# lh3/ksw2

Measured on AMD Instinct MI355X. Metric: GCUPS (DP cells/s) + pairs/s at fixed (qlen,tlen,band), higher is better.
Workload: dtype int16x2 (packed, two alignments per lane); 1 GPU; 10k: 49152 pairs/step/GPU, qlen=10000 tlen=10000 band=500 zdrop=400 extz2 affine score-only; setup_priming_batches=0, parallelism=pairs sharded over 1 GPU(s), one process per GPU, no collective in the data path

## Files before the change

### ksw2_amd/csrc/ksw2_host_plan.c

```c
#include "ksw2_host_int.h"


__thread char g_err[512];
__thread int g_no_defer;
static __thread int g_probe_tasks;
size_t thread_cached_device_bytes(void);

const char *ksw2amd_last_error(void) { return g_err; }
const char *ksw2amd_backend(void) { return k2a_shim_backend(); }
int ksw2amd_device_count(void) { return k2a_shim_device_count(); }


void ksw2amd_release_cache(void);

static const char *const g_env_name[ENV_COUNT] = {
#define X(n) "KSW2AMD_" #n,
	K2A_ENV_LIST
#undef X
};
__thread void *g_plan_stream;
__thread int g_latency_plan;
const char *g_env[ENV_COUNT];
volatile int g_env_ready;
static int g_env_gen;
// ... 234 lines not shown
	ez->n_cigar = 0; ez->zdropped = 0; ez->reach_end = 0;
}

void ez_reserve(void *km, ksw_extz_t *ez, int n)
{
	int m = ez->m_cigar;
	if (n <= m) return;
	while (m < n) m = m ? m << 1 : 4;
	ez->cigar = (uint32_t*)cigar_realloc(km, ez->cigar, (size_t)m << 2);
	ez->m_cigar = m;
}






int64_t band_cells(int qlen, int tlen, int w)
{
	const int64_t T = (int64_t)qlen + w < tlen ? (int64_t)qlen + w : tlen;
	const int64_t a = (int64_t)qlen - 1 - w;
	const int64_t na = a < 0 ? 0 : (a + 1 < T ? a + 1 : T);
	const int64_t nb = (int64_t)w + 1 < T ? (int64_t)w + 1 : T;
	const int64_t sum_en = na * (na - 1) / 2 + na * w + (T - na) * ((int64_t)qlen - 1);
	const int64_t sum_st = (T - nb) * (T - 1 + nb) / 2 - (T - nb) * (int64_t)w;
	return T <= 0 ? 0 : sum_en - sum_st + T;
}

static size_t mp_total_steps(int G, int C, int qlen, int tlen, int w)
{
	const int R = G * C, ngen = (tlen + R - 1) / R;
	size_t tot = 0;
	int g;
	for (g = 0; g < ngen; ++g) {
		const int lo = imax(0, g * R - w), hi = imin(qlen - 1, imin(g * R + R - 1, tlen - 1) + w);
		const int nl = imin(G, (tlen - g * R + C - 1) / C);
		if (hi >= lo) tot += ((size_t)(hi - lo + 1) + (size_t)(nl - 1) + 7) & ~(size_t)7;
		(void)0;
	}
	return tot;
}

int geom_fits(int G, int C, int tlen_eff, int w)
{
	const int nstrips = (tlen_eff + C - 1) / C;
	return nstrips <= G || 2 * (int64_t)w < (int64_t)G * (C + 1) - C + 1;
}

static int cfg_fits(int cfg, int tlen_eff, int w)
{
	if (cfg == K2A_CFG_MP) return 1;
	return geom_fits(k2a_cfg_G[cfg], k2a_cfg_C[cfg], tlen_eff, w);
}

void build_eff(int dual, int m, const int8_t *mat, int e, int e2, int generic, int8_t *eff)
{
	int a, b;
	if (generic) memcpy(eff, mat, (size_t)m * m);
	else {
		int scN = mat[m * m - 1] == 0 ? -(dual ? e2 : e) : mat[m * m - 1];
		for (a = 0; a < m; ++a)
			for (b = 0; b < m; ++b)
				eff[a * m + b] = (int8_t)((a == m - 1 || b == m - 1) ? scN : a == b ? mat[0] : mat[1]);
	}
}

static void build_scoring(int dual, int m, const int8_t *mat, int q, int e, int q2, int e2, int generic, K2aScoring *sc)
{
	int8_t eff[K2A_MAXM * K2A_MAXM];
	int a, b;
	memset(sc, 0, sizeof(*sc));
	sc->q = q; sc->e = e; sc->q2 = dual ? q2 : 0; sc->e2 = dual ? e2 : 0;
	sc->m = m;
	build_eff(dual, m, mat, e, e2, generic, eff);
	if (m > 5) return;
	for (a = 0; a < m; ++a) {
		uint32_t p = 0;
		for (b = 0; b < 4 && b < m; ++b) p |= (uint32_t)(uint8_t)eff[a * m + b] << (8 * b);
		sc->prof[a] = p;
		sc->colw[a] = m == 5 ? eff[a * m + 4] : 0;
	}
}

typedef struct { int ok, smax, smin, qemax, qemin, q, e, tn1; uint32_t cp[8]; } pkinfo_t;

static void pk_scoring(int dual, int m, const int8_t *mat, int q, int e, int q2, int e2, int generic, pkinfo_t *o)
{
	int8_t eff[25];
	int x, y, ok = (m >= 1 && m <= 5);
	memset(o, 0, sizeof(*o));
	if (ok) {
		build_eff(dual, m, mat, e, e2, generic, eff);
		o->smax = o->smin = eff[0];
		for (x = 0; x < m * m; ++x) { o->smax = imax(o->smax, eff[x]); o->smin = imin(o->smin, eff[x]); }
		for (y = 0; y < m; ++y)
			for (x = 0; x < 4 && x < m; ++x) o->cp[y] |= (uint32_t)(o->smax - eff[x * m + y]) << (8 * x);
		if (m == 5 && !(ENV(TN) && ENV(TN)[0] == '0')) {
			for (y = 1; y < 5 && eff[4 * 5 + y] == eff[4 * 5]; ++y) {}
			if (y == 5) o->tn1 = o->smax - eff[4 * 5] + 1;
		}
	}
	o->q = q; o->e = e;
	o->qemax = dual ? imax(q + e, q2 + e2) : q + e;
	o->qemin = dual ? imin(q + e, q2 + e2) : q + e;
	if (q < 0 || e < 0 || (dual && (q2 < 0 || e2 < 0)) || o->smax + e < 0) ok = 0;
	o->ok = ok;
}

static int pk_eligible(const pkinfo_t *k, int qlen, int tlen, int w)
{
	const int64_t L = imin(qlen, tlen);
	int64_t hmax, hmin;
	if (k->ok <= 0 || qlen > 32000 || tlen > 32000) return 0;
	hmax = (int64_t)imax(k->smax, 0) * L + (int64_t)k->e * tlen;
	hmin = -((int64_t)k->q + (int64_t)k->e * (w + 1)) + (int64_t)imin(k->smin, 0) * L;
	return hmax < K2A_PK_VMAX - 2 * k->qemax - 8 && hmin > K2A_NEG16 + 2 * k->qemax + 8;
}

static int pk_window_ok(const pkinfo_t *k, int qlen, int tlen, int w, int C)
{
	const int64_t D = imax(imax(k->smax, 0) + k->qemin, -k->smin) + k->e;
	if (k->ok <= 0 || qlen > 65000 || tlen > 65000) return 0;
	if ((int64_t)4 * C * D + 2 * k->qemax + imax(k->smax, 0) + (k->smax - k->smin) + 64 > K2A_PK_SLACK) return 0;
	return ((int64_t)2 * w + 2 * C + 2) * D + 2 * k->qemax + (int64_t)4 * C * D + 64 <= 12000;
}

static int pk_slide_ok(const pkinfo_t *k, int qlen, int tlen)
{
	const int64_t D = imax(imax(k->smax, 0) + k->qemin, -k->smin) + k->e;
	if (k->ok <= 0 || qlen > 65000 || tlen > 65000) return 0;
	if (K2A_PKMP_RMAX_LIMIT + (K2A_PKMP_T + 4) * D + 2 * k->qemax + 64 > K2A_PK_VMAX) return 0;
	return (K2A_PKMP_T + 2 * 16 + 4) * D + 2 * k->qemax + 64 <= 6000;
}

static inline uint64_t above4(uint64_t v) { return ((v >> 3 | v >> 4 | v >> 5 | v >> 6 | v >> 7) | ((v >> 2) & (v | (v >> 1)))) & 0x0101010101010101ull; }

int copy_scan(uint8_t *dst, const uint8_t *src, int n)
{
	int i = 0;
	uint64_t acc = 0, hi = 0, v0, v1, v2, v3;
	for (; i + 32 <= n; i += 32) {
		memcpy(&v0, src + i, 8); memcpy(&v1, src + i + 8, 8); memcpy(&v2, src + i + 16, 8); memcpy(&v3, src + i + 24, 8);
		memcpy(dst + i, &v0, 8); memcpy(dst + i + 8, &v1, 8); memcpy(dst + i + 16, &v2, 8); memcpy(dst + i + 24, &v3, 8);
		acc |= (v0 | v1) | (v2 | v3);
		if (((v0 | v1) | (v2 | v3)) & 0x0404040404040404ull) hi |= (above4(v0) | above4(v1)) | (above4(v2) | above4(v3));
	}
	for (; i < n; ++i) { dst[i] = src[i]; acc |= src[i]; if (src[i] > 4) hi = 1; }
	return (acc & 0xf8f8f8f8f8f8f8f8ull) || hi ? 2 : (acc & 0x0404040404040404ull) ? 1 : 0;
}

void ksw2amd_plan_destroy(ksw2amd_plan_t *p)
{
	int i;
	if (!p) return;
	if (p->gather) gather_wait(p);
	if (p->up_ev) { k2a_shim_event_sync(p->up_ev); k2a_shim_event_destroy(p->up_ev); p->up_ev = 0; }
	if (p->up_state) {
		int k;
		for (k = 0; k < K2A_MAXPIECES; ++k) if (p->up_state->ev2[k]) k2a_shim_event_destroy(p->up_state->ev2[k]);
		pthread_mutex_destroy(&p->up_state->mu); free(p->up_state); p->up_state = 0;
	}
	if (p->wm_ev) { k2a_shim_event_destroy(p->wm_ev); p->wm_ev = 0; }
	if (p->meta_ev) { k2a_shim_event_sync(p->meta_ev); k2a_shim_event_destroy(p->meta_ev); p->meta_ev = 0; }
	if (p->stream_used) k2a_shim_stream_sync(p->stream);
	cache_put(BUF_SEQ, p->d_seq, p->cap[BUF_SEQ]); cache_put(BUF_TB, p->d_tb, p->cap[BUF_TB]);
	if (p->meta_folded != 2) cache_put(BUF_PAIRS, p->d_pairs, p->cap[BUF_PAIRS]);
	cache_put(BUF_RES, p->d_res, p->cap[BUF_RES]);
	if (!p->meta_folded) cache_put(BUF_ORDER, p->d_order, p->cap[BUF_ORDER]);
	cache_put(BUF_CIG, p->d_cig, p->cap[BUF_CIG]);
	cache_put(BUF_BND, p->d_bnd, p->cap[BUF_BND]); cache_put(BUF_WM, p->d_wm, p->cap[BUF_WM]); cache_put(BUF_HMETA, p->h_meta, p->cap[BUF_HMETA]);
	cache_put(BUF_PK4, p->d_pk4, p->cap[BUF_PK4]);
	free(p->h_qd);
	for (i = 0; i < 3; ++i) if (p->ev[i]) { if (!g_ev_cache[i]) g_ev_cache[i] = p->ev[i]; else k2a_shim_event_destroy(p->ev[i]); }
	free(p->h_pairs); free(p->h_cls); free(p->h_half); free(p->h_flag); free(p->h_order);
	cache_put(BUF_HRES, p->h_res, p->cap[BUF_HRES]);
	if (!p->flat) cache_put(BUF_HSEQ, p->h_seq, p->cap[BUF_HSEQ]);
	free(p->src_pairs); free(p->src_mat); free(p->flat_tail); free(p->uni);
	free(p);
}

int cmp_cost_desc(const void *a, const void *b)
{
// ... 343 lines not shown
		const char *ev = ENV(SIMDS);
		const int simds = ev ? atoi(ev) : k2a_shim_simd_count();
		if (simds > 0) {
			int cnt[NCLS_MAX * NPASS], b;
			memset(cnt, 0, sizeof(cnt));
			if (uni) { if (p->h_cls[0] >= 0 && pk_ok[0] && pk_ok[0] != PASS_SOLO) cnt[p->h_cls[0] * NPASS + pk_ok[0]] = g_probe_tasks ? 2 * g_probe_tasks : n; }
			else
			for (i = 0; i < n; ++i) if (p->h_cls[i] >= 0 && pk_ok[i] && pk_ok[i] != PASS_SOLO) ++cnt[p->h_cls[i] * NPASS + pk_ok[i]];
			for (b = 0; b < NCLS_MAX * NPASS; ++b)
				if (cnt[b]) {
					const int pcb = (b % NPASS - 1) % K2A_NPKCFG, G = k2a_pkcfg_G[pcb];
					const int64_t waves = ((int64_t)(cnt[b] + 1) / 2 * G + 63) / 64 * (pcb == K2A_PKCFG_MP ? 4 : 1);
					cnt[b] = G != 64 ? 0 : (solo_mode == 3 && pcb != K2A_PKCFG_MP && cnt[b] <= simds ? 2 : 0) | (waves * 10 < (int64_t)simds * 4 ? 1 : 0);
				}
			if (uni && !(p->h_cls[0] >= 0 && pk_ok[0] && pk_ok[0] != PASS_SOLO && cnt[p->h_cls[0] * NPASS + pk_ok[0]])) {  }
			else
			for (i = 0; i < n; ++i)
				if (p->h_cls[i] >= 0 && pk_ok[i] && pk_ok[i] != PASS_SOLO) {
					const int what = cnt[p->h_cls[i] * NPASS + pk_ok[i]];
					if ((what & 2) && solo_ok[i]) pk_ok[i] = PASS_SOLO;
					else if (what & 1) pk_ok[i] = 0;
				}
		}
	}

	if (tlev) tph[3] = now_ms();
	if (m > 5 && !flat && !su) {
		build_eff(dual, m, sc->mat, e, e2, 0, (int8_t*)p->h_seq + mat_off);
		build_eff(dual, m, sc->mat, e, e2, 1, (int8_t*)p->h_seq + mat_off + (size_t)m * m);
	}
	if (!su && !g_probe_tasks) p->d_seq = (uint8_t*)cache_get(BUF_SEQ, p->seq_bytes + (flat ? 0 : META_ROOM(n)), &p->cap[BUF_SEQ]);
	if (!p->d_seq && !g_probe_tasks) { fail(KSW2AMD_E_NOMEM, "device allocation failed: %s", k2a_shim_last_error()); goto err; }
	up = su ? su->up : (flat && !flat->on_device) || (!flat && p->seq_bytes >= ((size_t)(ENV(SHARED_UP_MIN_MB) ? imax(atoi(ENV(SHARED_UP_MIN_MB)), 0) : 4) << 20) && !ENV(NO_SHARED_UP)) ? shared_upload_stream() : 0;
	if (up) shared_up = 1; else up = g_plan_stream ? g_plan_stream : thread_upload_stream();
	p->stream = up; p->stream_used = !g_probe_tasks;
	if (su) {  }
	else if (flat) {
		const size_t tail = p->seq_bytes - flat_span;
		flat_tmp = (uint8_t*)calloc(tail ? tail : 1, 1);
		if (!flat_tmp) { fail(KSW2AMD_E_NOMEM, "plan_create: host allocation failed%s", 0); goto err; }
		if (m > 5) {
			build_eff(dual, m, sc->mat, e, e2, 0, (int8_t*)flat_tmp + (mat_off - flat_span));
			build_eff(dual, m, sc->mat, e, e2, 1, (int8_t*)flat_tmp + (mat_off - flat_span) + (size_t)m * m);
		}
	}

	{
		enum { NB = NCLS_MAX * NPASS };
		int bcnt[NB], bpos[NB], b;
		p->ncls = 0; p->ntasks = 0;
		p->h_order = (uint32_t*)malloc(sizeof(uint32_t) * (3 * (size_t)n + 4));
		srt = (sort_t*)malloc(sizeof(sort_t) * ((size_t)n + 1));
		if (!p->h_order || !srt) { fail(KSW2AMD_E_NOMEM, "plan_create: host allocation failed%s", 0); goto err; }
		memset(bcnt, 0, sizeof(bcnt));
		if (uni) bcnt[p->h_cls[0] * NPASS + pk_ok[0]] = n;
		else
		for (i = 0; i < n; ++i) if (p->h_cls[i] >= 0) ++bcnt[p->h_cls[i] * NPASS + pk_ok[i]];
		for (b = 0, k = 0; b < NB; ++b) { bpos[b] = k; k += bcnt[b]; }
		if (uni) { for (b = 0; b < NB; ++b) bpos[b] += bcnt[b]; }
		else
		for (i = 0; i < n; ++i)
			if (p->h_cls[i] >= 0) {
				sort_t *e_ = &srt[bpos[p->h_cls[i] * NPASS + pk_ok[i]]++];
				e_->idx = (uint32_t)i;
				e_->cost = ((int64_t)p->h_pairs[i].qlen << 40) + ((int64_t)p->h_pairs[i].tlen << 16) + p->h_pairs[i].w;
				e_->tf = (uint32_t)p->h_pairs[i].tlen_full;
			}
		for (b = 0, k = 0; b < NB; ++b) {
			const int cnt = bcnt[b], pass = b % NPASS;
			sort_t *g = srt + (bpos[b] - cnt);
			int ntask = 0;
			cls_t *c;
			if (cnt == 0) continue;
			ci = b / NPASS;
			if (!uni) {
			for (i = 1; i < cnt && cmp_cost_desc(&g[i - 1], &g[i]) <= 0; ++i) {}
			if (i < cnt) qsort(g, (size_t)cnt, sizeof(sort_t), cmp_cost_desc);
			}
			c = &p->cls[p->ncls++];
			c->solo = pass == PASS_SOLO;
			c->cfg = c->solo ? 0 : pass ? (pass - 1) % K2A_NPKCFG : ci / 6; c->rb = pass && !c->solo ? ((pass - 1) / K2A_NPKCFG) & 1 : 0;
			c->nomax = !c->solo && pass > 2 * K2A_NPKCFG; c->mode = (ci / 2) % 3; c->generic = ci & 1; c->pk = pass != 0 && !c->solo; c->first = k;
			build_scoring(dual, m, sc->mat, q, e, q2, e2, c->generic, &c->sc);
			if (pkinfo[c->generic].ok > 0) { memcpy(c->sc.cp, pkinfo[c->generic].cp, sizeof(c->sc.cp)); c->sc.pk_smax = pkinfo[c->generic].smax; c->sc.pk_tn1 = pkinfo[c->generic].tn1; }
			if (uni) {
				if (!pass || c->solo) { for (i = 0; i < cnt; ++i) p->h_order[k++] = (uint32_t)i; ntask = cnt; }
				else for (i = 0; i < cnt; i += 2, ++ntask) { p->h_order[k++] = (uint32_t)i; p->h_order[k++] = (uint32_t)(i + 1 < cnt ? i + 1 : i); }
			} else
			if (!pass || c->solo) {
				for (i = 0; i < cnt; ++i) p->h_order[k++] = g[i].idx;
				ntask = cnt;
			} else {
				for (i = 0; i < cnt; ++ntask) {
					const uint32_t ia = g[i].idx;
					uint32_t ib = ia;
					if (i + 1 < cnt && g[i + 1].cost == g[i].cost && g[i + 1].tf == g[i].tf) { ib = g[i + 1].idx; i += 2; } else i += 1;
					p->h_order[k++] = ia; p->h_order[k++] = ib;
				}
			}
			c->count = ntask;
			p->ntasks += ntask;
		}
		p->norder = k;
		free(srt); srt = 0;
	}

	if (tlev) tph[4] = now_ms();
	for (k = 0; k < p->ncls; ++k) {
		const cls_t *c = &p->cls[k];
		if (!c->pk || c->cfg != K2A_PKCFG_MP) continue;
		for (i = 0; i < c->count; ++i) {
			K2aPair *da = &p->h_pairs[p->h_order[c->first + 2 * i]], *db = &p->h_pairs[p->h_order[c->first + 2 * i + 1]];
			p->bnd_words = align_up(p->bnd_words, 4);
			da->bnd_off = db->bnd_off = (uint32_t)p->bnd_words;
			p->bnd_words += align_up((size_t)da->qlen * (dual ? 5 : 4) + 16, 4) + K2A_PKMP_WAVES * (size_t)(64 * 16 * 2 * 2);
			if (p->bnd_words > 0xfff00000u) { fail(KSW2AMD_E_PARAM, "plan_create: boundary rows over 16 GiB in one plan%s", 0); goto err; }
		}
	}

	{
		const char *ev = ENV(DEFER);
		const int forced = ev && *ev ? (atoi(ev) != 0) : -1;
		size_t ck_total = 0;
		for (k = 0; k < p->ncls; ++k) {
			cls_t *c = &p->cls[k];
			c->defer = c->pk && !c->solo && c->cfg != K2A_PKCFG_MP && !dual && c->mode == K2A_MODE_SCORE && !c->nomax && !g_no_defer &&
			           (forced < 0 ? k2a_pkcfg_G[c->cfg] == 64 && (k2a_shim_simd_count() > 0 ? 2 * (int64_t)(g_probe_tasks ? g_probe_tasks : c->count) >= 3 * (int64_t)k2a_shim_simd_count()
			                                                                                      : (g_probe_tasks ? g_probe_tasks : c->count) >= 32) : forced);
		}
		if (g_probe_tasks) { free(pk_ok); free(solo_ok); return p; }
		for (lo = 0; lo < 2; ++lo) {
			size_t at = p->tb_bytes;
			for (k = 0; k < p->ncls; ++k) {
				const cls_t *c = &p->cls[k];
				const int G = c->pk ? k2a_pkcfg_G[c->cfg] : 64, C = c->pk ? k2a_pkcfg_C[c->cfg] : 16, NG = 64 / G;
				int t0;
				if (!c->defer) continue;
				at += align_up(4 * K2A_ZLIST_WORDS(c->count), 256);
				for (t0 = 0; t0 < c->count; t0 += NG) {
					uint32_t steps = 0, hs = 0;
					int t;
					size_t bytes;
					for (t = t0; t < imin(c->count, t0 + NG); ++t) {
						const K2aPair *d = &p->h_pairs[p->h_order[c->first + 2 * t]];
						const uint32_t ns = (uint32_t)((d->tlen + C - 1) / C);
						steps = (uint32_t)imax((int)steps, (int)ns - 1 + imin(d->qlen - 1, d->tlen - 1 + d->w) + 1);
						hs = (uint32_t)imax((int)hs, (int)ns);
					}
					bytes = align_up((size_t)steps * 512 + (size_t)NG * hs * 16, 256);
					if (lo) for (t = t0; t < imin(c->count, t0 + NG); ++t) {
						K2aPair *da = &p->h_pairs[p->h_order[c->first + 2 * t]], *db = &p->h_pairs[p->h_order[c->first + 2 * t + 1]];
						da->tb_off = db->tb_off = at; da->bnd_off = db->bnd_off = steps; da->cig_off = db->cig_off = hs;
					}
					at += bytes;
				}
			}
			if (!lo) {
				ck_total = at - p->tb_bytes;
				if (ck_total > ((size_t)1 << 30) && forced < 0) {
					size_t free_b = 0, total_b = 0;
					if (k2a_shim_mem_info(&free_b, &total_b) || ck_total > (free_b + thread_cached_device_bytes()) / 10 * 6) {
						for (k = 0; k < p->ncls; ++k) p->cls[k].defer = 0;
						ck_total = 0;
						break;
					}
				}
				if (ck_total == 0) break;
// ... 439 lines not shown
	}
	if (k2a_shim_event_record(p->ev[1], stream)) goto err;
	for (c = 0; c < p->ncls; ++c) {
		const cls_t *k = &p->cls[c];
		if (k->mode == K2A_MODE_SCORE || (streaming && k->qd >= 0)) continue;
		if (k->solo) {
			if (k2a_shim_launch_trace_solo(p->d_pairs, p->d_order + k->first, k->count, p->d_tb, p->d_res, p->d_cig, stream)) goto err;
		} else if (k->pk) {
			if (k2a_shim_launch_trace_pk(k->cfg, p->dual, p->d_pairs, p->d_order + k->first, k->count, p->d_tb, p->d_res, p->d_cig, stream)) goto err;
		} else if (k2a_shim_launch_trace(k->cfg, p->dual, p->d_pairs, p->d_order + k->first, k->count, p->d_tb, p->d_res, p->d_cig, stream)) goto err;
	}
	if (k2a_shim_event_record(p->ev[2], stream)) goto err;
	return KSW2AMD_OK;
err:
	return fail(KSW2AMD_E_NODEVICE, "plan_run: %s", k2a_shim_last_error());
}

int ksw2amd_plan_timing(ksw2amd_plan_t *p, float *fill_ms, float *total_ms)
{
	if (!p || !p->ran) return fail(KSW2AMD_E_PARAM, "plan_timing: plan has not run%s", 0);
	if (p->reject_all || p->ntasks == 0) { if (fill_ms) *fill_ms = 0; if (total_ms) *total_ms = 0; return KSW2AMD_OK; }
	if (fill_ms) *fill_ms = k2a_shim_event_ms(p->ev[0], p->ev[1]);
	if (total_ms) *total_ms = k2a_shim_event_ms(p->ev[0], p->ev[2]);
	return KSW2AMD_OK;
}

int64_t ksw2amd_plan_cells(const ksw2amd_plan_t *p) { return p ? p->cells : 0; }
int64_t ksw2amd_plan_packed_pairs(const ksw2amd_plan_t *p)
{
	int64_t n = 0;
	int c, i;
	if (!p) return 0;
	for (c = 0; c < p->ncls; ++c)
		if (p->cls[c].pk)
			for (i = 0; i < p->cls[c].count; ++i)
				n += p->h_order[p->cls[c].first + 2 * i] == p->h_order[p->cls[c].first + 2 * i + 1] ? 1 : 2;
		else if (p->cls[c].solo) n += p->cls[c].count;
	return n;
}
int ksw2amd_plan_describe(const ksw2amd_plan_t *p, char *buf, int cap)
{
	static const char *const mode_name[3] = { "score", "left", "right" }, *const form_name[4] = { "registers", "ldsrows", "ldscodes", "defer" };
	int c, len = 0;
	if (!p || !buf || cap <= 0) return 0;
	buf[0] = 0;
	if (p->splice == 2 && !p->reject_all) {
		static const char *const fkind[10] = { "extf-lds", "extf-lds", "extf-lds", "extf-hbm", "extf-win4", "extf-win8", "extf-lane", "extf-grp", "extf-grp32", "extf-grp64" };
		int nl = 0;
		for (c = 0; c < 10 && len < cap - 1; ++c)
			if (p->f_count[c]) {
				len += snprintf(buf + len, (size_t)(cap - len), "kernel=%s form=%s ring=%d tasks=%d\n", fkind[c], c == 6 && p->f_par.ring ? "ldsring" : c == 6 ? "hbm" : "-",
				                c == 6 ? p->f_par.ring : 0, p->f_count[c]);
				++nl;
			}
		return nl;
	}
	if (p->splice == 1 && !p->reject_all) {
		static const char *const skind[3] = { "exts-win8", "exts-win16", "exts-hbm" };
		int nl = 0, mode, g, wn;
		for (mode = 0; mode < 3; ++mode) for (g = 0; g < 2; ++g) for (wn = 0; wn < 3 && len < cap - 1; ++wn)
			if (p->s_count[mode][g][wn]) {
				len += snprintf(buf + len, (size_t)(cap - len), "kernel=%s mode=%s generic=%d tasks=%d\n", skind[wn], mode_name[mode], g, p->s_count[mode][g][wn]);
				++nl;
			}
		return nl;
	}
	if (p->splice == 3 && !p->reject_all) {
		static const char *const form_name[3] = { "hbm", "lds", "blk" };
		int nl = 0, mode, lds;
		for (mode = 0; mode < 3; ++mode) for (lds = 0; lds < 3 && len < cap - 1; ++lds)
			if (p->s_count[mode][0][lds]) {
				len += snprintf(buf + len, (size_t)(cap - len), "kernel=ssec gaps=%d mode=%s form=%s tasks=%d\n", p->dual ? 2 : 1, mode_name[mode], form_name[lds], p->s_count[mode][0][lds]);
				++nl;
			}
		return nl;
	}
	if (p->splice || p->reject_all) return 0;
	for (c = 0; c < p->ncls && len < cap - 1; ++c) {
		const cls_t *k = &p->cls[c];
		const char *kind = k->solo ? "solo" : k->pk ? (k->cfg == K2A_PKCFG_MP ? "pkmp" : "pk") : (k->cfg == K2A_CFG_MP ? "mp" : "int32");
		const int G = k->solo ? 64 : k->pk ? k2a_pkcfg_G[k->cfg] : k2a_cfg_G[k->cfg], C = k->solo ? 2 * K2A_SOLO_ROWS(k->mode == K2A_MODE_SCORE) : k->pk ? k2a_pkcfg_C[k->cfg] : k2a_cfg_C[k->cfg];
		const int form = k->defer ? 3 : k->solo ? 0 : k->pk ? (k->cfg == K2A_PKCFG_MP ? 0 : k2a_shim_pk_form(k->cfg, p->dual, k->mode, k->nomax, k->count))
		                                     : (k->cfg == K2A_CFG_MP ? k2a_shim_mp_form(p->dual, k->mode, k->count) : 0);
		len += snprintf(buf + len, (size_t)(cap - len), "kernel=%s G=%d C=%d gaps=%d mode=%s rebased=%d nomax=%d generic=%d form=%s tasks=%d uniform=%d wire4=%d tn=%d\n",
		                kind, G, C, p->dual ? 2 : 1, mode_name[k->mode], k->rb, k->nomax, k->generic, form_name[form], k->count, p->uni ? 1 : 0,
		                p->up_state ? p->up_state->wire4 : 0, (k->pk || k->solo) && k->sc.pk_tn1 ? 1 : 0);
	}
	return p->ncls;
}
int64_t ksw2amd_plan_device_bytes(const ksw2amd_plan_t *p)
{
	if (!p) return 0;
	return (int64_t)(p->seq_bytes + p->tb_bytes + p->cig_words * 4 + p->bnd_words * 4 + (sizeof(K2aPair) + sizeof(K2aResult)) * (size_t)p->n + 4 * (size_t)p->norder);
}

static int fetch_results(ksw2amd_plan_t *p)
{
	if (!p || !p->ran) return fail(KSW2AMD_E_PARAM, "plan_fetch: plan has not run%s", 0);
	if (p->gather && gather_wait(p)) return fail(KSW2AMD_E_NODEVICE, "plan_fetch: upload failed: %s", k2a_shim_last_error());
	if (p->reject_all || p->ntasks == 0) return KSW2AMD_OK;
	if (p->streamed && p->nqd > 0) {
		if (k2a_shim_stream_sync(p->stream)) return fail(KSW2AMD_E_NODEVICE, "plan_fetch: %s", k2a_shim_last_error());
		K2aQueueDesc back[NCLS_ENTRIES];
		int k, aborted = 0;
		if (k2a_shim_d2h(back, p->d_wm + K2A_WM_BYTES, sizeof(K2aQueueDesc) * (size_t)p->nqd, p->stream) || k2a_shim_stream_sync(p->stream))
			return fail(KSW2AMD_E_NODEVICE, "plan_fetch: %s", k2a_shim_last_error());
		for (k = 0; k < p->nqd; ++k) aborted |= back[k].abort != 0 || back[k].next < back[k].nwt;
		if (aborted) {
			void *st = p->stream;
			__sync_fetch_and_add(&g_stream_stat[1], 1);
			if (trace_level()) fprintf(stderr, "[ksw2_amd] streamed plan n=%d: a launch gave up waiting for its inputs (abort %u, started %u of %u wavefront-tasks, %d pieces); running the plan again behind its upload\n", p->n, back[0].abort, back[0].next, back[0].nwt, p->npieces);
			p->streamed = 0;
			if ((p->up_ev && k2a_shim_event_sync(p->up_ev)) || k2a_shim_memset(p->d_res, 0, sizeof(K2aResult) * (size_t)p->n, st) ||
			    (plan_wire4(p) && k2a_shim_launch_wire_expand(p->d_pk4, p->d_seq, (size_t)p->uni->n * p->uni->stride, plan_wire4(p), p->uni->stride, st)) ||
			    ksw2amd_plan_run(p, st) || k2a_shim_stream_sync(st))
				return fail(KSW2AMD_E_NODEVICE, "plan_fetch: %s", k2a_shim_last_error());
		}
	}
	if (k2a_shim_d2h(p->h_res, p->d_res, sizeof(K2aResult) * (size_t)p->n, p->stream) ||
	    k2a_shim_stream_sync(p->stream))
		return fail(KSW2AMD_E_NODEVICE, "plan_fetch: %s", k2a_shim_last_error());
	return KSW2AMD_OK;
}

int64_t g_reruns;
int64_t ksw2amd_rerun_count(void) { return g_reruns; }
int ksw2amd_plan_fetch_raw(ksw2amd_plan_t *p, int32_t *out16)
{
	int i, rc = fetch_results(p);
	if (rc) return rc;
	memset(out16, 0, sizeof(int32_t) * 16 * (size_t)p->n);
	for (i = 0; i < p->n; ++i)
		if (!p->reject_all && needs_rerun(p, i)) {
			ksw_extz_t z;
			int32_t *o = out16 + 16 * (size_t)i;
			memset(&z, 0, sizeof(z));
			rc = pair_rerun(p, i, 0, &z);
			if (rc) { free(z.cigar); return rc; }
			o[0] = (int32_t)z.max; o[1] = (int32_t)z.zdropped; o[2] = z.max_q; o[3] = z.max_t; o[4] = z.mqe; o[5] = z.mqe_t; o[6] = z.mte; o[7] = z.mte_q;
			o[8] = z.score; o[9] = z.reach_end; o[10] = z.n_cigar; o[11] = p->h_res[i].rows_done; o[12] = o[13] = -1;
			free(z.cigar);
		} else if (p->h_cls[i] >= 0 && !p->reject_all) memcpy(out16 + 16 * (size_t)i, &p->h_res[i], sizeof(K2aResult));
		else {
			int32_t *o = out16 + 16 * (size_t)i;
			o[2] = o[3] = o[5] = o[7] = -1; o[4] = o[6] = o[8] = KSW_NEG_INF; o[12] = o[13] = -1;
		}
	return KSW2AMD_OK;
}

void eqx_rewrite(void *km, const uint8_t *query, const uint8_t *target, int stride, ksw_extz_t *ez)
{
	int n0 = ez->n_cigar, k, i, x = 0, y = 0, n = 0;
	uint32_t *old = (uint32_t*)malloc(sizeof(uint32_t) * (size_t)(n0 + 1));
	memcpy(old, ez->cigar, sizeof(uint32_t) * (size_t)n0);
	ez->n_cigar = 0;
	for (k = 0; k < n0; ++k) {
		uint32_t op = old[k] & 0xf, len = old[k] >> 4;
		if (op == KSW_CIGAR_MATCH) {
			for (i = 0; i < (int)len; ++i) {
				uint32_t o = target[(size_t)(x + i) * stride] == query[(size_t)(y + i) * stride] ? KSW_CIGAR_EQ : KSW_CIGAR_X;
				if (n > 0 && (ez->cigar[n - 1] & 0xf) == o) ez->cigar[n - 1] += 1u << 4;
				else { ez_reserve(km, ez, n + 1); ez->cigar[n++] = 1u << 4 | o; }
			}
			x += (int)len; y += (int)len;
		} else {
			if (n > 0 && (ez->cigar[n - 1] & 0xf) == op) ez->cigar[n - 1] += len << 4;
			else { ez_reserve(km, ez, n + 1); ez->cigar[n++] = len << 4 | op; }
			if (op == KSW_CIGAR_DEL || op == KSW_CIGAR_N_SKIP) x += (int)len;
			else if (op == KSW_CIGAR_INS) y += (int)len;
// ... 292 lines not shown
```

### ksw2_amd/csrc/ksw2_lane_pk.h

```cpp
#ifndef KSW2_LANE_PK_H_
#define KSW2_LANE_PK_H_

#include "ksw2_lane.h"
#include "ksw2_lane_rowmask.h"

#define K2A_PK_STAGE(C) (3 * (C) + 4)
typedef uint32_t k2a_pk;
#define K2A_OFS   (K2A_OFS16 * 0x10001u)

K2A_FN k2a_pk k2a_pk2(int v) { return ((uint32_t)v & 0xffffu) | ((uint32_t)v << 16); }
K2A_FN int k2a_pk_lo(k2a_pk v) { return (int)(int16_t)(v & 0xffffu); }
K2A_FN int k2a_pk_hi(k2a_pk v) { return (int)(int16_t)(v >> 16); }
K2A_FN k2a_pk k2a_pk_sel(k2a_pk m, k2a_pk a, k2a_pk b) { return (m & a) | (~m & b); }
K2A_FN k2a_pk k2a_pair16(uint32_t lo, uint32_t hi) { return lo | (hi << 16); }
K2A_FN k2a_pk k2a_byte_pair(uint32_t a, uint32_t b, int r)
{
#if defined(__HIP_DEVICE_COMPILE__)
	return __builtin_amdgcn_perm(b, a, 0x0c040c00u + (uint32_t)r * 0x00010001u);
#else
	return ((a >> (8 * r)) & 0xffu) | (((b >> (8 * r)) & 0xffu) << 16);
#endif
}
K2A_FN uint32_t k2a_perm(uint32_t s0, uint32_t s1, uint32_t sel)
{
// ... 16 lines not shown
}
#define K2A_TSEL_BASE 0x0c040c00u
K2A_FN uint32_t k2a_h16(int v) { return (uint32_t)(v + K2A_OFS16) & 0xffffu; }
K2A_FN k2a_pk k2a_pku(int v) { return k2a_pk2(v + K2A_OFS16); }
K2A_FN k2a_pk k2a_add32(k2a_pk a, k2a_pk b) { return a + b; }
K2A_FN k2a_pk k2a_sub32(k2a_pk a, k2a_pk b) { return a - b; }

#if defined(__HIP_DEVICE_COMPILE__)
typedef short k2a_s2 __attribute__((ext_vector_type(2)));
typedef unsigned short k2a_u2 __attribute__((ext_vector_type(2)));
K2A_FN k2a_pk k2a_pk_add(k2a_pk a, k2a_pk b) { return __builtin_bit_cast(k2a_pk, (k2a_s2)(__builtin_bit_cast(k2a_s2, a) + __builtin_bit_cast(k2a_s2, b))); }
K2A_FN k2a_pk k2a_pk_sub(k2a_pk a, k2a_pk b) { return __builtin_bit_cast(k2a_pk, (k2a_s2)(__builtin_bit_cast(k2a_s2, a) - __builtin_bit_cast(k2a_s2, b))); }
K2A_FN k2a_pk k2a_pk_max(k2a_pk a, k2a_pk b) { return __builtin_bit_cast(k2a_pk, __builtin_elementwise_max(__builtin_bit_cast(k2a_s2, a), __builtin_bit_cast(k2a_s2, b))); }
K2A_FN k2a_pk k2a_pk_min(k2a_pk a, k2a_pk b) { return __builtin_bit_cast(k2a_pk, __builtin_elementwise_min(__builtin_bit_cast(k2a_s2, a), __builtin_bit_cast(k2a_s2, b))); }
K2A_FN k2a_pk k2a_pk_maxu(k2a_pk a, k2a_pk b) { return __builtin_bit_cast(k2a_pk, __builtin_elementwise_max(__builtin_bit_cast(k2a_u2, a), __builtin_bit_cast(k2a_u2, b))); }
K2A_FN k2a_pk k2a_pk_max3u(k2a_pk a, k2a_pk b, k2a_pk c)
{
	k2a_pk d;
	asm("v_pk_maximum3_f16 %0, %1, %2, %3" : "=v"(d) : "v"(a), "v"(b), "v"(c));
	return d;
}
K2A_FN k2a_pk k2a_pk_mad(k2a_pk a, k2a_pk b, k2a_pk c)
{
	k2a_pk d;
	asm("v_pk_mad_i16 %0, %1, %2, %3" : "=v"(d) : "v"(a), "v"(b), "v"(c));
	return d;
}
K2A_FN k2a_pk k2a_pk_sign(k2a_pk a)
{
	k2a_pk d;
	asm("v_pk_ashrrev_i16 %0, 15, %1 op_sel_hi:[0,1]" : "=v"(d) : "v"(a));
	return d;
}
K2A_FN k2a_pk k2a_pk_selv(k2a_pk m, k2a_pk a, k2a_pk b)
{
	k2a_pk d;
	asm("v_bitop3_b32 %0, %1, %2, %3 bitop3:0xe4" : "=v"(d) : "v"(a), "v"(b), "v"(m));
	return d;
}
K2A_FN k2a_pk k2a_pk_shl(k2a_pk a, int n)
{
	return n == 0 ? a : __builtin_bit_cast(k2a_pk, (k2a_u2)(__builtin_bit_cast(k2a_u2, a) << (k2a_u2)(unsigned short)n));
}
K2A_FN k2a_pk k2a_bit_mask(uint32_t bits, int c) { return (k2a_pk)__builtin_amdgcn_sbfe((int)bits, c, 1); }
#define K2A_SCHED_FENCE() __builtin_amdgcn_sched_barrier(0)
K2A_FN uint32_t k2a_load_early(const uint8_t *p) { uint32_t v; __builtin_memcpy(&v, p, 4); return v; }
#else
#define K2A_SCHED_FENCE() do {} while (0)
K2A_FN uint32_t k2a_load_early(const uint8_t *p) { uint32_t v; __builtin_memcpy(&v, p, 4); return v; }
K2A_FN k2a_pk k2a_pk_mk(int lo, int hi) { return ((uint32_t)lo & 0xffffu) | ((uint32_t)hi << 16); }
K2A_FN k2a_pk k2a_pk_add(k2a_pk a, k2a_pk b) { return k2a_pk_mk(k2a_pk_lo(a) + k2a_pk_lo(b), k2a_pk_hi(a) + k2a_pk_hi(b)); }
K2A_FN k2a_pk k2a_pk_sub(k2a_pk a, k2a_pk b) { return k2a_pk_mk(k2a_pk_lo(a) - k2a_pk_lo(b), k2a_pk_hi(a) - k2a_pk_hi(b)); }
K2A_FN k2a_pk k2a_pk_max(k2a_pk a, k2a_pk b) { return k2a_pk_mk(k2a_max(k2a_pk_lo(a), k2a_pk_lo(b)), k2a_max(k2a_pk_hi(a), k2a_pk_hi(b))); }
K2A_FN k2a_pk k2a_pk_min(k2a_pk a, k2a_pk b) { return k2a_pk_mk(k2a_min(k2a_pk_lo(a), k2a_pk_lo(b)), k2a_min(k2a_pk_hi(a), k2a_pk_hi(b))); }
K2A_FN k2a_pk k2a_pk_maxu(k2a_pk a, k2a_pk b)
{
	const uint32_t al = a & 0xffffu, ah = a >> 16, bl = b & 0xffffu, bh = b >> 16;
	return (al > bl ? al : bl) | ((ah > bh ? ah : bh) << 16);
}
K2A_FN k2a_pk k2a_pk_max3u(k2a_pk a, k2a_pk b, k2a_pk c)
{
	uint32_t r = 0;
	for (int h = 0; h < 2; ++h) {
		const uint32_t x = (a >> (16 * h)) & 0xffffu, y = (b >> (16 * h)) & 0xffffu, z = (c >> (16 * h)) & 0xffffu;
		uint32_t m = x > y ? x : y;
		m = m > z ? m : z;
		if (m > 0x7BFFu) m = 0x7BFFu - (m & 0xffu);
		r |= m << (16 * h);
	}
	return r;
}
K2A_FN k2a_pk k2a_pk_mad(k2a_pk a, k2a_pk b, k2a_pk c) { return k2a_pk_mk(k2a_pk_lo(a) * k2a_pk_lo(b) + k2a_pk_lo(c), k2a_pk_hi(a) * k2a_pk_hi(b) + k2a_pk_hi(c)); }
K2A_FN k2a_pk k2a_pk_sign(k2a_pk a) { return ((a & 0x8000u) ? 0xffffu : 0u) | ((a & 0x80000000u) ? 0xffff0000u : 0u); }
K2A_FN k2a_pk k2a_pk_selv(k2a_pk m, k2a_pk a, k2a_pk b) { return k2a_pk_sel(m, a, b); }
K2A_FN k2a_pk k2a_pk_shl(k2a_pk a, int n) { return (((a & 0xffffu) << n) & 0xffffu) | ((((a >> 16) << n) & 0xffffu) << 16); }
K2A_FN k2a_pk k2a_bit_mask(uint32_t bits, int c) { return ((bits >> c) & 1u) ? 0xffffffffu : 0u; }
#endif

K2A_FN uint32_t k2a_tsel_wild(uint32_t x)
{
	const uint32_t n = x & 0x00040004u;
	return ((x ^ n) + K2A_TSEL_BASE) | n | (n << 1);
}
K2A_FN k2a_pk k2a_tn_fix(k2a_pk cand, uint32_t sel, int tn1)
{
	const uint32_t m = (sel >> 3) & 0x00010001u;
	return cand - m * ((uint32_t)(tn1 - 1) & 0xffu);
}

#define K2A_SGN_SEL 0x09080b0au
template<bool DUAL, bool NIBBLE, bool INV>
K2A_FN uint32_t k2a_dir_flags(uint32_t s1, uint32_t s2, uint32_t s3, uint32_t s4, uint32_t x1, uint32_t x2, uint32_t x3, uint32_t x4)
{
	const uint32_t q1 = k2a_perm(s1, x1, K2A_SGN_SEL), q2 = k2a_perm(s2, x2, K2A_SGN_SEL);
	uint32_t r = k2a_pk_selv(0x55555555u, q1, q2);
	if (DUAL) {
		const uint32_t q3 = k2a_perm(s3, x3, K2A_SGN_SEL), q4 = k2a_perm(s4, x4, K2A_SGN_SEL);
		r = k2a_pk_selv(0x33333333u, r, k2a_pk_selv(0x55555555u, q3, q4));
	}
	if (INV) r = ~r;
	if (NIBBLE) return k2a_pk_selv(0x03030303u, r, r >> 16);
	const uint32_t t = k2a_pk_selv(0x0f0f0f0fu, r, r >> 16);
	return DUAL ? t : t & 0x33333333u;
}
K2A_FN uint32_t k2a_flags_decode(uint32_t b)
{
	const uint32_t win = (b & 8u) ? 4u : (b & 4u) ? 3u : (b & 2u) ? 2u : (b & 1u);
	return win | ((b >> 4) << 3);
}
K2A_FN k2a_pk k2a_ofs_on(k2a_pk plain) { return k2a_pk_add(plain, K2A_OFS); }
K2A_FN k2a_pk k2a_ofs_off(k2a_pk ofs) { return k2a_pk_sub(ofs, K2A_OFS); }

#define K2A_PK_LDSROWS(G, C, DUAL, MODE, NOMAX) ((G) == 64 && (C) == 16 && (DUAL) && (MODE) != K2A_MODE_SCORE && !(NOMAX))
#define K2A_PK_LDSROW_WORDS(C) (3 * (C) * 64)
#define K2A_PK_LDSCODES(G, C, DUAL, MODE, NOMAX) ((((G) == 64 && (C) == 16) || ((G) == 8 && (C) == 18) || ((G) == 16 && (C) == 8)) && !(DUAL) && (MODE) == K2A_MODE_SCORE)
#define K2A_PK_LDSCODE_WORDS(C) ((C) * 64)

struct K2aCkHead { int32_t baseA, baseB; uint32_t hd0, pad; };
#define K2A_CK_STEP_BYTES 512

struct K2aRowPredLane {
	uint32_t live;
	K2A_FN void begin(int dd, int w, int rows_m1)
	{
		const int lo = k2a_max(0, dd - w);
		const int hi = k2a_min(rows_m1, dd + w);
		const int cnt = k2a_max(hi - lo + 1, 0);
		live = ((1u << cnt) - 1u) << (lo & 31);
	}
	K2A_FN k2a_pk pick(int c, k2a_pk h, k2a_pk neg) const { return k2a_pk_sel(k2a_bit_mask(live, c), h, neg); }
	K2A_FN bool any() const { return live != 0; }
};
template<int C>
struct K2aRowPredUniform {
	const K2aRowMasks<C> &rm;
	int lane;
	K2A_FN K2aRowPredUniform(const K2aRowMasks<C> &rm_, int lane_) : rm(rm_), lane(lane_) {}
	K2A_FN void begin(int, int, int) {}
	K2A_FN k2a_pk pick(int c, k2a_pk h, k2a_pk neg) const
	{
#if defined(__HIP_DEVICE_COMPILE__)
		return __builtin_amdgcn_inverse_ballot_w64(rm.m[c]) ? h : neg;
#else
		return ((rm.m[c] >> lane) & 1u) ? h : neg;
#endif
	}
	K2A_FN bool any() const
	{
		uint64_t a = 0;
#pragma unroll
		for (int c = 0; c < C; ++c) a |= rm.m[c];
#if defined(__HIP_DEVICE_COMPILE__)
		return __builtin_amdgcn_inverse_ballot_w64(a);
#else
		return ((a >> lane) & 1u) != 0;
#endif
	}
};

template<int G, int C, bool DUAL, int MODE = K2A_MODE_SCORE, bool RB = false, bool NOMAX = false, int LDSROW_ = 0, bool DEFER = false, bool TN = false>
struct K2aLanePk {
	enum { NIB = K2A_PK_NIBBLES(C, DUAL), TBWORDS = NIB ? C / 4 : C / 2 };
	int qlen, tlen, tlen_full, w, nstrips;
	const uint8_t *qa, *qbp, *ta, *tbq;
	int gl, S, i0, je, koff, Snext, knext, koff_next;
	int kfin, kd, rows_m1, wup;
	k2a_pk hout, eout, e2out, hd0, hu_prev;
	int baseA, baseB;
	k2a_pk delta;
	uint32_t qb;
	uint32_t hasn;
	bool wn;
	const uint32_t *cptab;
	uint32_t cpA, cpB;
	K2A_FN void set_qb(uint32_t q) { qb = q; cpA = cptab[q & 7u]; cpB = cptab[(q >> 16) & 7u]; }
	enum { LDSROW = LDSROW_ == 1,
	       LDSTC = LDSROW_ != 0 };
	k2a_pk hl[C], f[C], f2[DUAL ? C : 1], rmax_[(NOMAX || LDSROW) ? 1 : C], rmj_[(NOMAX || LDSROW || DEFER) ? 1 : C];
	k2a_pk tc_[LDSTC ? 1 : C];
	uint32_t *lrow;
	enum { TCROW = LDSROW ? 2 : 0 };
	K2A_FN k2a_pk rmax(int c) const { return LDSROW ? lrow[(0 * C + c) * 64] : rmax_[(NOMAX || LDSROW) ? 0 : c]; }
	K2A_FN k2a_pk rmj(int c) const { return DEFER ? 0u : LDSROW ? lrow[(1 * C + c) * 64] : rmj_[(NOMAX || LDSROW) ? 0 : c]; }
	K2A_FN k2a_pk tc(int c) const { return LDSTC ? lrow[(TCROW * C + c) * 64] : tc_[LDSTC ? 0 : c]; }
	K2A_FN void set_rmax(int c, k2a_pk v) { if (LDSROW) lrow[(0 * C + c) * 64] = v; else rmax_[(NOMAX || LDSROW) ? 0 : c] = v; }
	K2A_FN void set_rmj(int c, k2a_pk v) { if (DEFER) return; if (LDSROW) lrow[(1 * C + c) * 64] = v; else rmj_[(NOMAX || LDSROW) ? 0 : c] = v; }
	K2A_FN void set_tc(int c, k2a_pk v) { if (LDSTC) lrow[(TCROW * C + c) * 64] = v; else tc_[LDSTC ? 0 : c] = v; }

	K2A_FN static int first_col(int S_, int w_) { return k2a_max(0, S_ * C - w_); }

	K2A_FN void schedule_next()
	{
		koff_next = Snext;
		knext = Snext < nstrips ? koff_next + first_col(Snext, w) : K2A_KNONE;
	}

	K2A_FN void setup(const K2aPair &pr, const K2aPair &prB, const uint8_t *seq, int lane_in_group, bool valid, const uint32_t *cptab_)
	{
		cptab = cptab_; cpA = cpB = 0;
		qlen = pr.qlen; tlen = pr.tlen; tlen_full = pr.tlen_full; w = pr.w;
		qa = seq + pr.qoff; ta = seq + pr.toff; qbp = seq + prB.qoff; tbq = seq + prB.toff;
		nstrips = valid ? (tlen + C - 1) / C : 0;
		gl = lane_in_group;
		S = -1; i0 = 0; je = -1; koff = 0; kfin = K2A_KNONE; kd = 0; rows_m1 = -1; wup = w;
		Snext = gl;
		schedule_next();
		const k2a_pk neg = k2a_pku(K2A_NEG16);
		hout = eout = e2out = hd0 = hu_prev = neg; qb = 0; qwA = qwB = 0; seen = 0;
		hasn = 0; wn = false;
		baseA = baseB = 0; delta = 0;
		local_reset();
#pragma unroll
		for (int c = 0; c < C; ++c) { hl[c] = f[c] = neg; set_tc(c, K2A_TSEL_BASE); if (!NOMAX) { set_rmax(c, neg); set_rmj(c, 0); } if (DUAL) f2[c] = neg; }
		if (NOMAX || LDSROW) rmax_[0] = neg;
		if (NOMAX || LDSROW || DEFER) rmj_[0] = 0;
		if (LDSTC) tc_[0] = 0;
		if (!DUAL) f2[0] = 0;
	}

	K2A_FN int last_step() const { return nstrips > 0 ? (nstrips - 1) + k2a_min(qlen - 1, tlen - 1 + w) : -1; }
	K2A_FN bool need_init(int k) const { return k == knext; }
	K2A_FN bool need_fin(int k) const { return k == kfin; }

	template<bool COL0U = false>
	K2A_FN void do_init(const K2aScoring &sc, int bsA = 0, int bsB = 0, const K2aCkHead *forced = 0, bool col0_any = true)
	{
		S = Snext; i0 = S * C; koff = koff_next;
		je = k2a_min(qlen - 1, k2a_min(i0 + C - 1, tlen - 1) + w);
		kfin = koff + je;
		kd = koff + i0;
		rows_m1 = k2a_min(C - 1, tlen - 1 - i0);
		wup = w + (S == 0 ? 1 : 0);
		const int js = k2a_max(0, i0 - w);
		const k2a_pk neg = k2a_pku(K2A_NEG16);
		const uint8_t *tpa = ta + (size_t)S * C, *tpb = tbq + (size_t)S * C;
		hasn = 0;
#pragma unroll
		for (int c4 = 0; c4 < C; c4 += 4) {
			uint32_t da, db;
			__builtin_memcpy(&da, tpa + c4, 4); __builtin_memcpy(&db, tpb + c4, 4);
			if (c4 + 4 > C) { da &= 0xffffu; db &= 0xffffu; }
			note_codes(da, db);
			if (TN && sc.pk_tn1 && ((da | db) & 0x04040404u)) {
				hasn = 1;
#pragma unroll
				for (int r = 0; r < 4 && c4 + r < C; ++r) set_tc(c4 + r, k2a_tsel_wild(k2a_byte_pair(da, db, r)));
			} else {
#pragma unroll
				for (int r = 0; r < 4 && c4 + r < C; ++r) set_tc(c4 + r, k2a_byte_pair(da, db, r) + K2A_TSEL_BASE);
			}
		}
#pragma unroll
		for (int c = 0; c < C; ++c) {
			hl[c] = neg; f[c] = neg; if (DUAL) f2[c] = neg;
			if (!NOMAX) set_rmax(c, neg);
		}
		const int hcorner = k2a_border<DUAL>(sc, i0) + sc.e * (i0 - 1);
		if (forced) { baseA = forced->baseA; baseB = forced->baseB; delta = 0; }
		else if (RB) {
			const int nbA = js == 0 ? hcorner : bsA + k2a_pk_lo(k2a_ofs_off(hu_prev)), nbB = js == 0 ? hcorner : bsB + k2a_pk_hi(k2a_ofs_off(hu_prev));
			delta = S == 0 ? 0u : k2a_pair16((uint32_t)(bsA - nbA) & 0xffffu, (uint32_t)(bsB - nbB) & 0xffffu);
			baseA = nbA; baseB = nbB;
		}
		if (col0_any) {
			if (COL0U) K2A_SCHED_FENCE();
			if (i0 <= w) {
#pragma unroll
				for (int c = 0; c < C; ++c) {
					const int hb = k2a_border<DUAL>(sc, i0 + c + 1) + sc.e * (i0 + c);
					if (i0 + c <= w) {
						hl[c] = k2a_ofs_on(k2a_pair16((uint32_t)(hb - baseA) & 0xffffu, (uint32_t)(hb - baseB) & 0xffffu));
						f[c] = k2a_pk_sub(hl[c], k2a_pk2(sc.q + sc.e));
						if (DUAL) f2[c] = k2a_pk_sub(hl[c], k2a_pk2(sc.q2 + sc.e2));
					}
				}
			}
		}
		if (forced) hd0 = forced->hd0;
		else if (RB) hd0 = K2A_OFS;
		else if (js == 0) hd0 = k2a_pku(hcorner);
		else hd0 = hu_prev;
		Snext += G;
		schedule_next();
	}

	K2A_FN void top_inputs(const K2aScoring &sc, int k, k2a_pk &hin, k2a_pk &ein, k2a_pk &e2in) const
	{
		if (S == 0) {
			const int hb = k2a_border<DUAL>(sc, k - koff + 1);
			const k2a_pk h0 = k2a_ofs_on(k2a_pair16((uint32_t)(hb - baseA) & 0xffffu, (uint32_t)(hb - baseB) & 0xffffu));
			hin = k2a_pk_sub(h0, k2a_pk2(sc.e));
			ein = k2a_pk_sub(h0, k2a_pk2(sc.q + sc.e)); e2in = k2a_pk_sub(h0, k2a_pk2(sc.q2 + sc.e2));
		}
	}

	K2A_FN bool step(const K2aScoring &sc, int k, k2a_pk hin, k2a_pk ein, k2a_pk e2in, uint32_t *tbw)
	{
		K2aRowPredLane rp;
		return step_rows(sc, k, hin, ein, e2in, tbw, rp);
	}

	template<class RowPred>
	K2A_FN bool step_rows(const K2aScoring &sc, int k, k2a_pk hin, k2a_pk ein, k2a_pk e2in, uint32_t *tbw, RowPred &rp)
	{
		const int dd = k - kd;
		const k2a_pk neg = k2a_pku(K2A_NEG16);
		const k2a_pk gq = k2a_pk2(sc.q), ge = k2a_pk2(sc.e), gq2 = k2a_pk2(sc.q2), ge2 = k2a_pk2(sc.e2), de2 = k2a_pk2(sc.e2 - sc.e);
		const k2a_pk bias = k2a_pk2(sc.pk_smax + sc.e);
		k2a_pk e = ein, e2 = e2in;
		if (dd >= wup) { e = neg; e2 = neg; }
		rp.begin(dd, w, rows_m1);
		const k2a_pk jjpk = k2a_pk2(k - koff);
		constexpr int CH = (C % 6 == 0) ? 6 : (C % 4 == 0) ? 4 : C;
		k2a_pk dprev = 0, uprev = 0, above_old = hd0;
#pragma unroll
		for (int c0 = 0; c0 < C; c0 += CH) {
			k2a_pk cand[CH];
			const k2a_pk last_old = hl[c0 + CH - 1];
#pragma unroll
			for (int r = 0; r < CH; ++r) {
				const int c = c0 + r;
				const k2a_pk up = r == 0 ? above_old : hl[c - 1];
				cand[r] = k2a_sub32(k2a_add32(up, bias), k2a_perm(cpB, cpA, tc(c)));
			}
			if (TN && wn) {
#pragma unroll
				for (int r = 0; r < CH; ++r) cand[r] = k2a_tn_fix(cand[r], tc(c0 + r), sc.pk_tn1);
			}
			above_old = last_old;
			if (CH < C) K2A_SCHED_FENCE();
#pragma unroll
			for (int r = 0; r < CH; ++r) {
				const int c = c0 + r;
				const k2a_pk fc = f[c];
				k2a_pk h = cand[r], s1 = 0, s2 = 0, s3 = 0, s4 = 0, x1 = 0, x2 = 0, x3 = 0, x4 = 0;
				if (MODE == K2A_MODE_SCORE) {
					h = k2a_pk_max3u(h, e, fc);
					if (DUAL) h = k2a_pk_max3u(h, e2, f2[c]);
				} else if (MODE == K2A_MODE_LEFT) {
					s1 = k2a_pk_sub(h, e);  h = k2a_pk_maxu(h, e);
					s2 = k2a_pk_sub(h, fc); h = k2a_pk_maxu(h, fc);
					if (DUAL) { s3 = k2a_pk_sub(h, e2); h = k2a_pk_maxu(h, e2); s4 = k2a_pk_sub(h, f2[c]); h = k2a_pk_maxu(h, f2[c]); }
				} else {
					s1 = k2a_pk_sub(e, h);  h = k2a_pk_maxu(h, e);
					s2 = k2a_pk_sub(fc, h); h = k2a_pk_maxu(h, fc);
					if (DUAL) { s3 = k2a_pk_sub(e2, h); h = k2a_pk_maxu(h, e2); s4 = k2a_pk_sub(f2[c], h); h = k2a_pk_maxu(h, f2[c]); }
				}
				h = rp.pick(c, h, neg);
				if (!NOMAX && DEFER) set_rmax(c, k2a_pk_maxu(rmax(c), h));
				else if (!NOMAX) {
					const k2a_pk rm = rmax(c), rj = rmj(c);
					if (!DUAL && MODE == K2A_MODE_RIGHT) set_rmj(c, k2a_pk_selv(k2a_pk_sign(k2a_pk_sub(rm, h)), jjpk, rj));
					else set_rmj(c, k2a_pk_selv(k2a_pk_sign(k2a_pk_sub(h, rm)), rj, jjpk));
					set_rmax(c, k2a_pk_maxu(rm, h));
				}
				const k2a_pk t = k2a_sub32(h, gq);
				if (MODE == K2A_MODE_LEFT) { x1 = k2a_pk_sub(t, e); x2 = k2a_pk_sub(t, fc); }
				else if (MODE == K2A_MODE_RIGHT) { x1 = k2a_pk_sub(e, t); x2 = k2a_pk_sub(fc, t); }
				e = k2a_pk_maxu(e, t);
				f[c] = k2a_sub32(k2a_pk_maxu(fc, t), ge);
				if (DUAL) {
					const k2a_pk t2 = k2a_sub32(h, gq2);
					if (MODE == K2A_MODE_LEFT) { x3 = k2a_pk_sub(t2, e2); x4 = k2a_pk_sub(t2, f2[c]); }
					else if (MODE == K2A_MODE_RIGHT) { x3 = k2a_pk_sub(e2, t2); x4 = k2a_pk_sub(f2[c], t2); }
					e2 = k2a_pk_sub(k2a_pk_maxu(e2, t2), de2);
					f2[c] = k2a_sub32(k2a_pk_maxu(f2[c], t2), ge2);
				}
				if (MODE != K2A_MODE_SCORE) {
					const uint32_t fl = k2a_dir_flags<DUAL, NIB != 0, MODE == K2A_MODE_RIGHT>(s1, s2, s3, s4, x1, x2, x3, x4);
					if (!(c & 1)) dprev = fl;
					else if (NIB) {
						const uint32_t u = k2a_pk_selv(0x0f0f0f0fu, dprev, fl << 4);
						if ((c & 3) == 3) tbw[c >> 2] = k2a_perm(u, uprev, 0x05010400u);
						else uprev = u;
					} else tbw[c >> 1] = k2a_perm(fl, dprev, 0x05040100u);
				}
				hl[c] = h;
			}
			if (CH < C) K2A_SCHED_FENCE();
		}
		hd0 = hin;
		hout = hl[C - 1]; eout = e; e2out = e2;
		return rp.any();
	}

	K2A_FN uint32_t next_query_codes(int k) const
	{
		const int j = k + 1 - ((k + 1 == knext) ? koff_next : koff);
		const int jc = k2a_min(k2a_max(j, 0), qlen - 1);
		return k2a_pair16(qa[jc], qbp[jc]);
	}

	uint32_t qwA, qwB;
	uint32_t seen;
	K2A_FN void load_query_group(int kg, int koff_use, uint32_t &a, uint32_t &b)
	{
		const int jc = k2a_min(k2a_max(kg - koff_use, 0), qlen - 1);
		a = k2a_load_early(qa + jc); b = k2a_load_early(qbp + jc);
	}
	K2A_FN void note_codes(uint32_t a, uint32_t b) { seen |= a | b; }
	K2A_FN bool saw_wildcard() const { return (seen & 0xfcfcfcfcu) != 0; }
	K2A_FN void reload_query_group(int k)
	{
		const int j = (k & ~3) - koff;
		const int sh = 8 * k2a_min(k2a_max(-j, 0), 3);
		uint32_t va, vb;
		load_query_group(k & ~3, koff, va, vb);
		qwA = va << sh; qwB = vb << sh;
	}
	K2A_FN static uint32_t query_pick(uint32_t a, uint32_t b, int kk)
	{
#if defined(__HIP_DEVICE_COMPILE__)
		return __builtin_amdgcn_perm(b, a, 0x0c040c00u + (uint32_t)kk * 0x00010001u);
#else
		return k2a_byte_pair(a, b, kk);
#endif
	}

	K2A_FN void stage_rows(uint32_t *rowbuf) const
	{
#pragma unroll
		for (int c = 0; c < C; ++c) { rowbuf[c] = k2a_ofs_off(hl[c]); rowbuf[C + c] = k2a_ofs_off(rmax(c)); rowbuf[2 * C + c] = rmj(c); }
		rowbuf[3 * C] = (uint32_t)i0;
		if (RB) { rowbuf[3 * C + 1] = (uint32_t)baseA; rowbuf[3 * C + 2] = (uint32_t)baseB; }
	}

	K2A_FN void do_fin_seq(const K2aScoring &sc, K2aBook *bA, K2aBook *bB, int zdropA, int zdropB, const uint32_t *rowbuf)
	{
		const int zslope = DUAL ? sc.e2 : sc.e;
#pragma nounroll
		for (int half = 0; half < 2; ++half) {
			K2aBook *b = half ? bB : bA;
			const int zdrop = half ? zdropB : zdropA;
			const int sh = half ? 16 : 0;
			int bmax = b->max, bmax_t = b->max_t, bmax_q = b->max_q, bmqe = b->mqe, bmqe_t = b->mqe_t;
			int bmte = b->mte, bmte_q = b->mte_q, bscore = b->score, bdrop = b->dropped, brows = b->rows;
#pragma nounroll
			for (int c = 0; c < C; ++c) {
				const int i = i0 + c;
				if (i < tlen && !bdrop) {
					const bool reach = i + w >= qlen - 1;
					const int unb = (half ? baseB : baseA) - sc.e * i;
					const int hend = (int)(int16_t)(rowbuf[c] >> sh) + unb, H = (int)(int16_t)(rowbuf[C + c] >> sh) + unb;
					const int j = (int)(uint16_t)(rowbuf[2 * C + c] >> sh);
					if (reach && hend > bmqe) { bmqe = hend; bmqe_t = i; }
					if (i == tlen_full - 1) { bmte = H; bmte_q = j; }
					if (H > bmax) { bmax = H; bmax_t = i; bmax_q = j; }
					else if (DEFER) {
						if (zdrop >= 0 && bmax - H > zdrop) { bdrop = 1; b->inexact = 1; }
					} else if (i >= bmax_t && j >= bmax_q) {
						const int dt = i - bmax_t, dq = j - bmax_q;
						const int skew = dt > dq ? dt - dq : dq - dt;
						if (zdrop >= 0 && bmax - H > zdrop + skew * zslope) bdrop = 1;
					}
					if (!bdrop && i == tlen_full - 1 && reach) bscore = hend;
					brows = i + 1;
				}
			}
			b->max = bmax; b->max_t = bmax_t; b->max_q = bmax_q; b->mqe = bmqe; b->mqe_t = bmqe_t;
			b->mte = bmte; b->mte_q = bmte_q; b->score = bscore; b->dropped = bdrop; b->rows = brows;
		}
		end_strip();
	}

	K2A_FN bool fin_fast(const K2aScoring &sc, K2aBook *bA, K2aBook *bB, int zdropA, int zdropB)
	{
		if (i0 + C >= tlen || i0 + C - 1 + w >= qlen - 1) return false;
		k2a_pk m = k2a_ofs_off(rmax(0)), mn = m, arg = 0, argj = rmj(0);
#pragma unroll
		for (int c = 1; c < (NOMAX ? 1 : C); ++c) {
			const k2a_pk v = k2a_pk_sub(rmax(c), k2a_pk2(sc.e * c + K2A_OFS16));
			const k2a_pk gt = k2a_pk_sign(k2a_pk_sub(m, v));
			arg = k2a_pk_sel(gt, k2a_pk2(c), arg);
			argj = k2a_pk_sel(gt, rmj(c), argj);
			m = k2a_pk_max(m, v);
			mn = k2a_pk_min(mn, v);
		}
		const int offA = (RB ? baseA : 0) - sc.e * i0, offB = (RB ? baseB : 0) - sc.e * i0;
		const int MA = k2a_pk_lo(m) + offA, MB = k2a_pk_hi(m) + offB, mA = k2a_pk_lo(mn) + offA, mB = k2a_pk_hi(mn) + offB;
		const int bmA = bA->max, bmB = bB->max;
		const bool deadA = bA->dropped != 0, deadB = bB->dropped != 0;
		if (!deadA && zdropA >= 0 && k2a_max(bmA, MA) - mA > zdropA) return false;
		if (!deadB && zdropB >= 0 && k2a_max(bmB, MB) - mB > zdropB) return false;
		if (!deadA) {
			if (MA > bmA) { bA->max = MA; bA->max_t = i0 + k2a_pk_lo(arg); bA->max_q = (int)(argj & 0xffffu); }
			bA->rows = i0 + C;
		}
		if (!deadB) {
			if (MB > bmB) { bB->max = MB; bB->max_t = i0 + k2a_pk_hi(arg); bB->max_q = (int)(argj >> 16); }
			bB->rows = i0 + C;
		}
		end_strip();
		return true;
	}

	k2a_pk lmax, lmax_t, lmax_q, lmqe, lmqe_t;
	k2a_pk last_h, last_m, last_j;

	K2A_FN void local_reset()
	{
		lmax = 0; lmax_t = lmax_q = 0xffffffffu; lmqe = k2a_pk2(K2A_NEG16); lmqe_t = 0xffffffffu;
		last_h = last_m = last_j = 0;
	}

	K2A_FN void fin_local_rows(const K2aScoring &sc, const uint32_t *rowbuf)
	{
		const int fi0 = (int)rowbuf[3 * C];
#pragma nounroll
		for (int c = gl; c < C; c += G) {
			const int i = fi0 + c;
			const k2a_pk bias = k2a_pk2(sc.e * i);
			const k2a_pk pj = rowbuf[2 * C + c], ipk = k2a_pk2(i);
			const k2a_pk ph = (i < tlen) ? k2a_pk_sub(rowbuf[c], bias) : k2a_pk2(K2A_NEG16);
			const k2a_pk pm = (i < tlen) ? k2a_pk_sub(rowbuf[C + c], bias) : k2a_pk2(K2A_NEG16);
			const k2a_pk up = k2a_pk_sign(k2a_pk_sub(lmax, pm));
			lmax_t = k2a_pk_sel(up, ipk, lmax_t);
			lmax_q = k2a_pk_sel(up, pj, lmax_q);
			lmax = k2a_pk_max(lmax, pm);
			const k2a_pk reach = (i + w >= qlen - 1) ? 0xffffffffu : 0u;
			const k2a_pk uq = k2a_pk_sign(k2a_pk_sub(lmqe, ph)) & reach;
			lmqe_t = k2a_pk_sel(uq, ipk, lmqe_t);
			lmqe = k2a_pk_sel(uq, ph, lmqe);
			if (i == tlen_full - 1 && tlen == tlen_full) { last_h = ph; last_m = pm; last_j = pj; }
		}
	}
	K2A_FN void end_strip() { S = -1; je = -1; kfin = K2A_KNONE; rows_m1 = -1; hasn = 0; }

	K2A_FN void fin_score_only(const K2aScoring &sc, K2aBook *bA, K2aBook *bB)
	{
		const int last = tlen_full - 1;
		if (tlen == tlen_full && last >= i0 && last < i0 + C && last + w >= qlen - 1) {
			k2a_pk v = 0;
#pragma unroll
			for (int c = 0; c < C; ++c) if (i0 + c == last) v = k2a_ofs_off(hl[c]);
			bA->score = k2a_pk_lo(v) + (RB ? baseA : 0) - sc.e * last;
			bB->score = k2a_pk_hi(v) + (RB ? baseB : 0) - sc.e * last;
		}
		end_strip();
	}
};

template<int C>
K2A_FN void k2a_fin_rows_half(const K2aScoring &sc, K2aBook *b, int zdrop, const uint32_t *rowbuf, int half, bool rb, int qlen, int tlen, int tlen_full, int w)
{
	const int i0 = (int)rowbuf[3 * C], base = rb ? (int)rowbuf[3 * C + 1 + half] : 0, sh = half ? 16 : 0;
	int bmax = b->max, bmax_t = b->max_t, bmax_q = b->max_q, bmqe = b->mqe, bmqe_t = b->mqe_t;
	int bmte = b->mte, bmte_q = b->mte_q, bscore = b->score, bdrop = b->dropped, brows = b->rows;
#pragma nounroll
	for (int c = 0; c < C; ++c) {
		const int i = i0 + c;
		if (i < tlen && !bdrop) {
			const bool reach = i + w >= qlen - 1;
			const int unb = base - sc.e * i;
			const int hend = (int)(int16_t)(rowbuf[c] >> sh) + unb, H = (int)(int16_t)(rowbuf[C + c] >> sh) + unb;
			const int j = (int)(uint16_t)(rowbuf[2 * C + c] >> sh);
			if (reach && hend > bmqe) { bmqe = hend; bmqe_t = i; }
			if (i == tlen_full - 1) { bmte = H; bmte_q = j; }
			if (H > bmax) { bmax = H; bmax_t = i; bmax_q = j; }
			else if (i >= bmax_t && j >= bmax_q) {
				const int dt = i - bmax_t, dq = j - bmax_q;
				const int skew = dt > dq ? dt - dq : dq - dt;
				if (zdrop >= 0 && bmax - H > zdrop + skew * sc.e) bdrop = 1;
			}
			if (!bdrop && i == tlen_full - 1 && reach) bscore = hend;
			brows = i + 1;
		}
	}
	b->max = bmax; b->max_t = bmax_t; b->max_q = bmax_q; b->mqe = bmqe; b->mqe_t = bmqe_t;
	b->mte = bmte; b->mte_q = bmte_q; b->score = bscore; b->dropped = bdrop; b->rows = brows;
}

template<int G, int C, bool DUAL = true, bool MP = false>
K2A_FN int k2a_trace_pair_pk(const uint8_t *tb, int half, int i, int j, uint32_t *out, int qlen, int tlen, int w, uint8_t *win)
{
	return k2a_trace_walk<G, C, K2A_PK_NIBBLES(C, DUAL) ? 3 : 2, MP>(tb, half, i, j, out, qlen, tlen, w, win);
}

K2A_FN void k2a_merge_local(const uint32_t *loc, int G, int half, K2aBook *b)
{
	int bmax = 0, bmax_t = -1, bmax_q = -1, bmqe = K2A_NEG, bmqe_t = -1;
	for (int l = 0; l < G; ++l) {
		const uint32_t *r = loc + l * 5;
		const int m = half ? k2a_pk_hi(r[0]) : k2a_pk_lo(r[0]);
		const int mt = half ? k2a_pk_hi(r[1]) : k2a_pk_lo(r[1]);
		const int mq = half ? k2a_pk_hi(r[2]) : k2a_pk_lo(r[2]);
		const int qe = half ? k2a_pk_hi(r[3]) : k2a_pk_lo(r[3]);
		const int qt = half ? k2a_pk_hi(r[4]) : k2a_pk_lo(r[4]);
		if (mt >= 0 && (m > bmax || (m == bmax && bmax_t >= 0 && mt < bmax_t))) { bmax = m; bmax_t = mt; bmax_q = mq; }
		if (qt >= 0 && (qe > bmqe || (qe == bmqe && qt < bmqe_t))) { bmqe = qe; bmqe_t = qt; }
	}
	b->max = bmax; b->max_t = bmax_t; b->max_q = bmax_q; b->mqe = bmqe; b->mqe_t = bmqe_t;
}

#endif
```

### ksw2_amd/csrc/ksw2_lane_pkmp.h

```cpp
#ifndef KSW2_LANE_PKMP_H_
#define KSW2_LANE_PKMP_H_

#include "ksw2_lane_pk.h"
#include "ksw2_shim.h"

#define K2A_PKMP_SPILL_WORDS(C) (64 * (C) * 2 * 2)
#define K2A_PKMP_BND_WORDS(qlen, dual) ((((size_t)(qlen) * ((dual) ? 5 : 4) + 16) + 3) & ~(size_t)3)

#if defined(__HIP_DEVICE_COMPILE__)
K2A_FN void k2a_key_max(unsigned long long *slot, unsigned long long key)
{
	__hip_atomic_fetch_max(slot, key, __ATOMIC_RELAXED, __HIP_MEMORY_SCOPE_WORKGROUP);
}
K2A_FN unsigned long long k2a_key_load(const unsigned long long *slot)
{
	return __hip_atomic_load(slot, __ATOMIC_RELAXED, __HIP_MEMORY_SCOPE_AGENT);
}
#else
K2A_FN void k2a_key_max(unsigned long long *slot, unsigned long long key) { if (key > *slot) *slot = key; }
K2A_FN unsigned long long k2a_key_load(const unsigned long long *slot) { return *slot; }
#endif

template<int C, bool DUAL, int MODE, bool TN = false>
struct K2aLanePkMp {
// ... 26 lines not shown
	K2A_FN bool need_init(int k) const { return k == P.knext; }
	K2A_FN bool need_fin(int k) const { return k == P.kfin; }
	K2A_FN int column(int k) const { return k - P.koff; }
	K2A_FN void do_init(const K2aScoring &sc, int bsA, int bsB)
	{
		P.do_init(sc, bsA, bsB);
		P.knext = K2A_KNONE;
	}
	K2A_FN void refresh_delta(int bsA, int bsB)
	{
		P.delta = k2a_pair16((uint32_t)(bsA - P.baseA) & 0xffffu, (uint32_t)(bsB - P.baseB) & 0xffffu);
	}
	K2A_FN k2a_pk adopt(k2a_pk raw) const
	{
		const k2a_pk dead = k2a_pk_sign(k2a_pk_sub(raw, k2a_pku(K2A_PKMP_DEAD)));
		return k2a_pk_sel(dead, k2a_pku(K2A_NEG16), k2a_pk_add(raw, P.delta));
	}

	K2A_FN static k2a_pk shift(k2a_pk v, k2a_pk d)
	{
		const k2a_pk s = k2a_pk_sub(v, d);
		const k2a_pk dead = k2a_pk_sign(k2a_pk_sub(s, k2a_pku(K2A_PKMP_DEAD)));
		return k2a_pk_sel(dead, k2a_pku(K2A_NEG16), s);
	}

	K2A_FN void flush_rowmax()
	{
#pragma unroll
		for (int c = 0; c < C; ++c) {
			const k2a_pk m = k2a_ofs_off(P.rmax(c)), j = P.rmj(c);
			const int mA = k2a_pk_lo(m), mB = k2a_pk_hi(m);
			const uint32_t jA = j & 0xffffu, jB = j >> 16;
			if (mA > K2A_PKMP_DEAD) k2a_key_max(&spill[2 * c], ((unsigned long long)((uint32_t)(mA + P.baseA) ^ 0x80000000u) << 32) | (FIRSTJ ? 0xffffu - jA : jA));
			if (mB > K2A_PKMP_DEAD) k2a_key_max(&spill[2 * c + 1], ((unsigned long long)((uint32_t)(mB + P.baseB) ^ 0x80000000u) << 32) | (FIRSTJ ? 0xffffu - jB : jB));
			P.set_rmax(c, k2a_pku(K2A_NEG16)); P.set_rmj(c, 0);
		}
	}

	K2A_FN k2a_pk rebase()
	{
		k2a_pk m = P.hl[0];
#pragma unroll
		for (int c = 1; c < C; ++c) m = k2a_pk_maxu(m, P.hl[c]);
		m = k2a_ofs_off(m);
		const k2a_pk dead = k2a_pk_sign(k2a_pk_sub(m, k2a_pk2(K2A_PKMP_DEAD)));
		const k2a_pk d = k2a_pk_sel(dead, 0u, m);
		k2a_pk over = 0;
#pragma unroll
		for (int c = 0; c < C; ++c) over |= k2a_pk_sign(k2a_pk_sub(k2a_pk2(K2A_PKMP_RMAX_LIMIT), k2a_pk_sub(k2a_ofs_off(P.rmax(c)), d)));
		if (over != 0) flush_rowmax();
		P.baseA += k2a_pk_lo(d); P.baseB += k2a_pk_hi(d);
#pragma unroll
		for (int c = 0; c < C; ++c) {
			P.hl[c] = shift(P.hl[c], d); P.f[c] = shift(P.f[c], d); if (DUAL) P.f2[c] = shift(P.f2[c], d);
			P.set_rmax(c, shift(P.rmax(c), d));
		}
		P.hd0 = shift(P.hd0, d); P.hout = shift(P.hout, d); P.eout = shift(P.eout, d);
		if (DUAL) P.e2out = shift(P.e2out, d);
		return d;
	}
	K2A_FN void after_rebase(k2a_pk d_above, int bsA, int bsB)
	{
		P.hu_prev = shift(P.hu_prev, d_above);
		refresh_delta(bsA, bsB);
	}

	K2A_FN void do_fin(const K2aScoring &sc, K2aBook *bA, K2aBook *bB, int zdropA, int zdropB, uint32_t *rowbuf)
	{
		const int zslope = DUAL ? sc.e2 : sc.e;
#pragma unroll
		for (int c = 0; c < C; ++c) rowbuf[c] = k2a_ofs_off(P.hl[c]);
#pragma nounroll
		for (int half = 0; half < 2; ++half) {
			K2aBook *b = half ? bB : bA;
			const int zdrop = half ? zdropB : zdropA, base = half ? P.baseB : P.baseA, sh = half ? 16 : 0;
			int bmax = b->max, bmax_t = b->max_t, bmax_q = b->max_q, bmqe = b->mqe, bmqe_t = b->mqe_t;
			int bmte = b->mte, bmte_q = b->mte_q, bscore = b->score, bdrop = b->dropped, brows = b->rows;
#pragma nounroll
			for (int c = 0; c < C; ++c) {
				const int i = P.i0 + c;
				if (i < P.tlen && !bdrop) {
					const bool reach = i + P.w >= P.qlen - 1;
					const unsigned long long key = k2a_key_load(&spill[2 * c + half]);
					const int hend = (int)(int16_t)(rowbuf[c] >> sh) + base - sc.e * i;
					const int H = (int)((uint32_t)(key >> 32) ^ 0x80000000u) - sc.e * i;
					const int j = FIRSTJ ? 0xffff - (int)(key & 0xffffu) : (int)(key & 0xffffu);
					if (reach && hend > bmqe) { bmqe = hend; bmqe_t = i; }
					if (i == P.tlen_full - 1) { bmte = H; bmte_q = j; }
					if (H > bmax) { bmax = H; bmax_t = i; bmax_q = j; }
					else if (i >= bmax_t && j >= bmax_q) {
						const int dt = i - bmax_t, dq = j - bmax_q;
						const int skew = dt > dq ? dt - dq : dq - dt;
						if (zdrop >= 0 && bmax - H > zdrop + skew * zslope) bdrop = 1;
					}
					if (!bdrop && i == P.tlen_full - 1 && reach) bscore = hend;
					brows = i + 1;
				}
			}
			b->max = bmax; b->max_t = bmax_t; b->max_q = bmax_q; b->mqe = bmqe; b->mqe_t = bmqe_t;
			b->mte = bmte; b->mte_q = bmte_q; b->score = bscore; b->dropped = bdrop; b->rows = brows;
		}
		P.end_strip();
	}
};

K2A_FN int k2a_pkmp_lag(int jlo_p, int jlo_c) { return (jlo_c - jlo_p + K2A_PKMP_T + K2A_PKMP_T - 1) / K2A_PKMP_T + 1; }

#endif
```

### ksw2_amd/csrc/ksw2_lane_solo.h

```cpp
#ifndef KSW2_LANE_SOLO_H_
#define KSW2_LANE_SOLO_H_

#include "ksw2_lane_pk.h"

#define K2A_SOLO_STAGE(C) (6 * (C) + 4)

template<int C>
K2A_FN size_t k2a_solo_steps(int qlen, int tlen, int w)
{
	const int nds = (tlen + 2 * C - 1) / (2 * C);
	return nds > 0 ? (size_t)(2 * (nds - 1) + 2 + k2a_min(qlen - 1, tlen - 1 + w)) : 0;
}

template<int C, bool DUAL, int MODE = K2A_MODE_SCORE, bool TN = false>
struct K2aLaneSolo {
	enum { G = 64, TBWORDS = C / 2 };
	int qlen, tlen, tlen_full, w, nds;
	const uint8_t *qa, *ta;
	int gl, D, i0, koff, Dnext, knext, koff_next;
	int kfin, kfinA, kd, kB0, rowsA_m1, rowsB_m1, wupA;
	k2a_pk hout, eout, e2out, hd0, hu_prev;
	int baseA, baseB;
	k2a_pk delta;
	uint32_t qb, qw;
	uint32_t tnA[(C + 3) / 4], tnB[(C + 3) / 4], qn0;
	int qn_sh;
	const uint32_t *cptab;
	uint32_t cpA, cpB;
	uint32_t seen;
	uint32_t hasn;
	bool wn;
	K2A_FN void note_codes(uint32_t a) { seen |= a; }
	K2A_FN bool saw_wildcard() const { return (seen & 0xfcfcfcfcu) != 0; }
	k2a_pk hl[C], f[C], f2[DUAL ? C : 1], rmax[C], rmj[C], tc[C], hsave[C];

	K2A_FN static int first_col(int D_, int w_) { return k2a_max(0, D_ * 2 * C - w_); }
	K2A_FN void schedule_next()
	{
		koff_next = 2 * Dnext;
		knext = Dnext < nds ? koff_next + first_col(Dnext, w) : K2A_KNONE;
	}

	K2A_FN void prefetch_next()
	{
		qn_sh = 0;
		if (Dnext < nds) {
			const uint8_t *tp = ta + (size_t)Dnext * 2 * C;
#pragma unroll
			for (int x = 0; x < (C + 3) / 4; ++x) { tnA[x] = k2a_load_early(tp + 4 * x); tnB[x] = k2a_load_early(tp + C + 4 * x); }
			const int j = (knext & ~3) - koff_next;
			qn_sh = 8 * k2a_min(k2a_max(-j, 0), 3);
			qn0 = k2a_load_early(qa + k2a_min(k2a_max(j, 0), qlen - 1));
		}
	}

	K2A_FN void setup(const K2aPair &pr, const uint8_t *seq, int lane, bool valid, const uint32_t *cptab_)
	{
		cptab = cptab_; cpA = cpB = 0;
		qlen = pr.qlen; tlen = pr.tlen; tlen_full = pr.tlen_full; w = pr.w;
		qa = seq + pr.qoff; ta = seq + pr.toff;
		nds = valid ? (tlen + 2 * C - 1) / (2 * C) : 0;
		gl = lane;
		D = -1; i0 = 0; koff = 0; kfin = kfinA = K2A_KNONE; kd = 0; kB0 = 0; rowsA_m1 = rowsB_m1 = -1; wupA = w;
		Dnext = gl;
		schedule_next();
#pragma unroll
		for (int x = 0; x < (C + 3) / 4; ++x) tnA[x] = tnB[x] = 0;
		qn0 = 0; seen = 0; hasn = 0; wn = false;
		prefetch_next();
		const k2a_pk neg = k2a_pku(K2A_NEG16);
		hout = eout = e2out = hd0 = hu_prev = neg; qb = 0; qw = 0; baseA = baseB = 0; delta = 0;
#pragma unroll
		for (int c = 0; c < C; ++c) { hl[c] = f[c] = rmax[c] = hsave[c] = neg; rmj[c] = 0; tc[c] = K2A_TSEL_BASE; if (DUAL) f2[c] = neg; }
		if (!DUAL) f2[0] = 0;
	}

	K2A_FN int last_step() const
	{
		if (nds <= 0) return -1;
		const int Dl = nds - 1, rB = tlen - 1 - (Dl * 2 * C + C);
		return rB >= 0 ? 2 * Dl + 1 + k2a_min(qlen - 1, tlen - 1 + w) : 2 * Dl + k2a_min(qlen - 1, tlen - 1 + w);
	}
	K2A_FN bool need_init(int k) const { return k == knext; }
	K2A_FN bool need_fin(int k) const { return k == kfin; }
	K2A_FN bool need_save(int k) const { return k == kfinA; }

	K2A_FN void do_init(const K2aScoring &sc, int bs)
	{
		D = Dnext; i0 = D * 2 * C; koff = koff_next;
		const int i0b = i0 + C;
		rowsA_m1 = k2a_min(C - 1, tlen - 1 - i0);
		rowsB_m1 = k2a_max(-1, k2a_min(C - 1, tlen - 1 - i0b));
		const int jeA = k2a_min(qlen - 1, k2a_min(i0 + C - 1, tlen - 1) + w);
		const int jeB = k2a_min(qlen - 1, k2a_min(i0b + C - 1, tlen - 1) + w);
		kfinA = koff + jeA;
		kfin = rowsB_m1 >= 0 ? koff + 1 + jeB : kfinA;
		kd = koff + i0;
		kB0 = rowsB_m1 >= 0 ? koff + 1 + k2a_max(0, i0b - w) : K2A_KNONE;
		wupA = w + (D == 0 ? 1 : 0);
		const int js = k2a_max(0, i0 - w);
		const k2a_pk neg = k2a_pku(K2A_NEG16);
		hasn = 0;
#pragma unroll
		for (int c4 = 0; c4 < C; c4 += 4) {
			const uint32_t da = tnA[c4 / 4], db = tnB[c4 / 4];
			note_codes(da | db);
			if (TN && sc.pk_tn1 && ((da | db) & 0x04040404u)) {
				hasn = 1;
#pragma unroll
				for (int r = 0; r < 4; ++r) tc[c4 + r] = k2a_tsel_wild(k2a_byte_pair(da, db, r));
			} else {
#pragma unroll
				for (int r = 0; r < 4; ++r) tc[c4 + r] = k2a_byte_pair(da, db, r) + K2A_TSEL_BASE;
			}
		}
#pragma unroll
		for (int c = 0; c < C; ++c) { hl[c] = neg; f[c] = neg; if (DUAL) f2[c] = neg; rmax[c] = neg; rmj[c] = 0; }
		const int hcorner = k2a_border<DUAL>(sc, i0) + sc.e * (i0 - 1);
		const int nb = js == 0 ? hcorner : bs + k2a_pk_hi(k2a_ofs_off(hu_prev));
		delta = D == 0 ? 0u : ((uint32_t)(bs - nb) & 0xffffu);
		baseA = nb;
		if (i0 <= w) {
#pragma unroll
			for (int c = 0; c < C; ++c) {
				const int ha = k2a_border<DUAL>(sc, i0 + c + 1) + sc.e * (i0 + c);
				const uint32_t va = i0 + c <= w ? k2a_h16(ha - baseA) : k2a_h16(K2A_NEG16);
				hl[c] = k2a_pair16(va, neg >> 16);
				const k2a_pk fl = k2a_pk_sub(hl[c], k2a_pk2(sc.q + sc.e));
				f[c] = k2a_pair16(i0 + c <= w ? fl & 0xffffu : neg & 0xffffu, neg >> 16);
				if (DUAL) {
					const k2a_pk fl2 = k2a_pk_sub(hl[c], k2a_pk2(sc.q2 + sc.e2));
					f2[c] = k2a_pair16(i0 + c <= w ? fl2 & 0xffffu : neg & 0xffffu, neg >> 16);
				}
			}
		}
		hd0 = k2a_pair16(k2a_h16(0), neg >> 16);
		qw = qn0 << qn_sh;
		Dnext += G;
		schedule_next();
		prefetch_next();
	}

	K2A_FN bool need_init_high(int k) const { return k == kB0; }

	K2A_FN void start_high(const K2aScoring &sc)
	{
		const int i0b = i0 + C;
		if (i0b <= w) {
			const uint32_t negh = (uint32_t)k2a_h16(K2A_NEG16);
			baseB = k2a_border<DUAL>(sc, i0b) + sc.e * (i0b - 1);
#pragma unroll
			for (int c = 0; c < C; ++c) {
				const bool in = i0b + c <= w;
				const int hb = k2a_border<DUAL>(sc, i0b + c + 1) + sc.e * (i0b + c) - baseB;
				const uint32_t vb = in ? k2a_h16(hb) : negh;
				const uint32_t fb = in ? k2a_h16(hb - (sc.q + sc.e)) : negh;
				hl[c] = (hl[c] & 0xffffu) | (vb << 16);
				f[c] = (f[c] & 0xffffu) | (fb << 16);
				if (DUAL) {
					const uint32_t fb2 = in ? k2a_h16(hb - (sc.q2 + sc.e2)) : negh;
					f2[c] = (f2[c] & 0xffffu) | (fb2 << 16);
				}
			}
		} else baseB = baseA + k2a_pk_hi(k2a_ofs_off(hd0));
		hd0 = (hd0 & 0xffffu) | ((uint32_t)k2a_h16(0) << 16);
		delta = (delta & 0xffffu) | (((uint32_t)(baseA - baseB) & 0xffffu) << 16);
	}

	K2A_FN void top_inputs(const K2aScoring &sc, int k, k2a_pk &hin, k2a_pk &ein, k2a_pk &e2in) const
	{
		if (D == 0) {
			const int hb = k2a_border<DUAL>(sc, k - koff + 1) - baseA;
			const uint32_t h0 = k2a_h16(hb - sc.e), e0 = k2a_h16(hb - (sc.q + sc.e));
			const uint32_t e20 = k2a_h16(hb - (sc.q2 + sc.e2));
			hin = (hin & 0xffff0000u) | h0; ein = (ein & 0xffff0000u) | e0; e2in = (e2in & 0xffff0000u) | e20;
		}
	}

	K2A_FN bool step(const K2aScoring &sc, int k, k2a_pk hin, k2a_pk ein, k2a_pk e2in, uint32_t *tbw)
	{
		const int ddA = k - kd, ddB = ddA - C - 1;
		const k2a_pk neg = k2a_pku(K2A_NEG16);
		const k2a_pk gq = k2a_pk2(sc.q), ge = k2a_pk2(sc.e), gq2 = k2a_pk2(sc.q2), ge2 = k2a_pk2(sc.e2), de2 = k2a_pk2(sc.e2 - sc.e);
		const k2a_pk bias = k2a_pk2(sc.pk_smax + sc.e);
		const k2a_pk cut = k2a_pair16(ddA >= wupA ? 0xffffu : 0u, ddB >= w ? 0xffffu : 0u);
		k2a_pk e = k2a_pk_sel(cut, neg, ein), e2 = DUAL ? k2a_pk_sel(cut, neg, e2in) : 0u;
		const int loA = k2a_max(0, ddA - w), hiA = k2a_min(rowsA_m1, ddA + w), cntA = k <= kfinA ? k2a_max(hiA - loA + 1, 0) : 0;
		const int loB = k2a_max(0, ddB - w), hiB = k2a_min(rowsB_m1, ddB + w), cntB = k >= kB0 ? k2a_max(hiB - loB + 1, 0) : 0;
		const uint32_t liveA = ((1u << cntA) - 1u) << (loA & 31), liveB = ((1u << cntB) - 1u) << (loB & 31);
		const uint32_t lv = liveA | (liveB << 16);
		const k2a_pk jjpk = k2a_pair16((uint32_t)(k - koff) & 0xffffu, (uint32_t)(k - koff - 1) & 0xffffu);
		constexpr int CH = (MODE != K2A_MODE_SCORE && C % 4 == 0) ? 4 : C;
		k2a_pk dprev = 0, above_old = hd0;
#pragma unroll
		for (int c0 = 0; c0 < C; c0 += CH) {
			k2a_pk cand[CH];
			const k2a_pk last_old = hl[c0 + CH - 1];
#pragma unroll
			for (int r = 0; r < CH; ++r) {
				const int c = c0 + r;
				cand[r] = k2a_sub32(k2a_add32(r == 0 ? above_old : hl[c - 1], bias), k2a_perm(cpB, cpA, tc[c]));
			}
			if (TN && wn) {
#pragma unroll
				for (int r = 0; r < CH; ++r) cand[r] = k2a_tn_fix(cand[r], tc[c0 + r], sc.pk_tn1);
			}
			above_old = last_old;
			if (CH < C) K2A_SCHED_FENCE();
#pragma unroll
			for (int r = 0; r < CH; ++r) {
				const int c = c0 + r;
				const k2a_pk fc = f[c];
				k2a_pk h = cand[r], s1 = 0, s2 = 0, s3 = 0, s4 = 0, x1 = 0, x2 = 0, x3 = 0, x4 = 0;
				if (MODE == K2A_MODE_SCORE) {
					h = k2a_pk_max3u(h, e, fc);
					if (DUAL) h = k2a_pk_max3u(h, e2, f2[c]);
				} else if (MODE == K2A_MODE_LEFT) {
					s1 = k2a_pk_sub(h, e);  h = k2a_pk_maxu(h, e);
					s2 = k2a_pk_sub(h, fc); h = k2a_pk_maxu(h, fc);
					if (DUAL) { s3 = k2a_pk_sub(h, e2); h = k2a_pk_maxu(h, e2); s4 = k2a_pk_sub(h, f2[c]); h = k2a_pk_maxu(h, f2[c]); }
				} else {
					s1 = k2a_pk_sub(e, h);  h = k2a_pk_maxu(h, e);
					s2 = k2a_pk_sub(fc, h); h = k2a_pk_maxu(h, fc);
					if (DUAL) { s3 = k2a_pk_sub(e2, h); h = k2a_pk_maxu(h, e2); s4 = k2a_pk_sub(f2[c], h); h = k2a_pk_maxu(h, f2[c]); }
				}
				h = k2a_pk_sel(k2a_pk_sign(lv << (15 - c)), h, neg);
				if (!DUAL && MODE == K2A_MODE_RIGHT) rmj[c] = k2a_pk_selv(k2a_pk_sign(k2a_pk_sub(rmax[c], h)), jjpk, rmj[c]);
				else rmj[c] = k2a_pk_selv(k2a_pk_sign(k2a_pk_sub(h, rmax[c])), rmj[c], jjpk);
				rmax[c] = k2a_pk_maxu(rmax[c], h);
				const k2a_pk t = k2a_sub32(h, gq);
				if (MODE == K2A_MODE_LEFT) { x1 = k2a_pk_sub(t, e); x2 = k2a_pk_sub(t, fc); }
				else if (MODE == K2A_MODE_RIGHT) { x1 = k2a_pk_sub(e, t); x2 = k2a_pk_sub(fc, t); }
				e = k2a_pk_maxu(e, t);
				f[c] = k2a_sub32(k2a_pk_maxu(fc, t), ge);
				if (DUAL) {
					const k2a_pk t2 = k2a_sub32(h, gq2);
					if (MODE == K2A_MODE_LEFT) { x3 = k2a_pk_sub(t2, e2); x4 = k2a_pk_sub(t2, f2[c]); }
					else if (MODE == K2A_MODE_RIGHT) { x3 = k2a_pk_sub(e2, t2); x4 = k2a_pk_sub(f2[c], t2); }
					e2 = k2a_pk_sub(k2a_pk_maxu(e2, t2), de2);
					f2[c] = k2a_sub32(k2a_pk_maxu(f2[c], t2), ge2);
				}
				if (MODE != K2A_MODE_SCORE) {
					const uint32_t fl = k2a_dir_flags<DUAL, false, MODE == K2A_MODE_RIGHT>(s1, s2, s3, s4, x1, x2, x3, x4);
					if (c & 1) tbw[c >> 1] = k2a_perm(fl, dprev, 0x05040100u);
					else dprev = fl;
				}
				hl[c] = h;
			}
			if (CH < C) K2A_SCHED_FENCE();
		}
		hd0 = hin;
		hout = hl[C - 1]; eout = e; e2out = e2;
		return (liveA | liveB) != 0;
	}

	K2A_FN void load_query_group(int kg, int koff_use, uint32_t &a) const
	{
		const int jc = k2a_min(k2a_max(kg - koff_use, 0), qlen - 1);
		a = k2a_load_early(qa + jc);
	}
	K2A_FN void advance_query(int kk)
	{
#if defined(__HIP_DEVICE_COMPILE__)
		qb = __builtin_amdgcn_perm(qb, qw, 0x0c040c00u + (uint32_t)kk);
#else
		qb = ((qw >> (8 * kk)) & 0xffu) | ((qb & 0xffu) << 16);
#endif
		cpB = cpA; cpA = cptab[qb & 7u];
	}

	K2A_FN void save_low() {
#pragma unroll
		for (int c = 0; c < C; ++c) hsave[c] = hl[c];
	}

	K2A_FN void stage_rows(uint32_t *rowbuf) const
	{
#pragma unroll
		for (int c = 0; c < C; ++c) {
			const k2a_pk hA = k2a_ofs_off(rowsB_m1 >= 0 ? hsave[c] : hl[c]), hB = k2a_ofs_off(hl[c]), m = k2a_ofs_off(rmax[c]);
			rowbuf[c] = hA & 0xffffu; rowbuf[C + c] = hB >> 16;
			rowbuf[2 * C + c] = m & 0xffffu; rowbuf[3 * C + c] = m >> 16;
			rowbuf[4 * C + c] = rmj[c] & 0xffffu; rowbuf[5 * C + c] = rmj[c] >> 16;
		}
	}

	K2A_FN void do_fin_seq(const K2aScoring &sc, K2aBook *b, int zdrop, const uint32_t *rowbuf)
	{
		const int zslope = DUAL ? sc.e2 : sc.e;
		int bmax = b->max, bmax_t = b->max_t, bmax_q = b->max_q, bmqe = b->mqe, bmqe_t = b->mqe_t;
		int bmte = b->mte, bmte_q = b->mte_q, bscore = b->score, bdrop = b->dropped, brows = b->rows;
#pragma nounroll
		for (int c = 0; c < 2 * C; ++c) {
			const int i = i0 + c;
			if (i < tlen && !bdrop) {
				const bool reach = i + w >= qlen - 1;
				const int unb = (c < C ? baseA : baseB) - sc.e * i;
				const int hend = (int)(int16_t)rowbuf[c] + unb, H = (int)(int16_t)rowbuf[2 * C + c] + unb;
				const int j = (int)(uint16_t)rowbuf[4 * C + c];
				if (reach && hend > bmqe) { bmqe = hend; bmqe_t = i; }
				if (i == tlen_full - 1) { bmte = H; bmte_q = j; }
				if (H > bmax) { bmax = H; bmax_t = i; bmax_q = j; }
				else if (i >= bmax_t && j >= bmax_q) {
					const int dt = i - bmax_t, dq = j - bmax_q;
					const int skew = dt > dq ? dt - dq : dq - dt;
					if (zdrop >= 0 && bmax - H > zdrop + skew * zslope) bdrop = 1;
				}
				if (!bdrop && i == tlen_full - 1 && reach) bscore = hend;
				brows = i + 1;
			}
		}
		b->max = bmax; b->max_t = bmax_t; b->max_q = bmax_q; b->mqe = bmqe; b->mqe_t = bmqe_t;
		b->mte = bmte; b->mte_q = bmte_q; b->score = bscore; b->dropped = bdrop; b->rows = brows;
		end_strip();
	}

	K2A_FN bool fin_fast(const K2aScoring &sc, K2aBook *b, int zdrop)
	{
		if (i0 + 2 * C >= tlen || i0 + 2 * C - 1 + w >= qlen - 1) return false;
		const k2a_pk hb = k2a_pair16(0u, (uint32_t)(sc.e * C) & 0xffffu);
		k2a_pk m = k2a_pk_sub(k2a_ofs_off(rmax[0]), hb), mn = m, arg = 0, argj = rmj[0];
#pragma unroll
		for (int c = 1; c < C; ++c) {
			const k2a_pk v = k2a_pk_sub(k2a_pk_sub(k2a_ofs_off(rmax[c]), hb), k2a_pk2(sc.e * c));
			const k2a_pk gt = k2a_pk_sign(k2a_pk_sub(m, v));
			arg = k2a_pk_sel(gt, k2a_pk2(c), arg);
			argj = k2a_pk_sel(gt, rmj[c], argj);
			m = k2a_pk_max(m, v);
			mn = k2a_pk_min(mn, v);
		}
		const int offA = baseA - sc.e * i0, offB = baseB - sc.e * i0;
		const int MA = k2a_pk_lo(m) + offA, MB = k2a_pk_hi(m) + offB;
		const int mnn = k2a_min(k2a_pk_lo(mn) + offA, k2a_pk_hi(mn) + offB);
		const int M = k2a_max(MA, MB), bm = b->max;
		if (b->dropped) { end_strip(); return true; }
		if (zdrop >= 0 && k2a_max(bm, M) - mnn > zdrop) return false;
		if (M > bm) {
			if (MB > MA) { b->max = MB; b->max_t = i0 + C + k2a_pk_hi(arg); b->max_q = (int)(argj >> 16); }
			else { b->max = MA; b->max_t = i0 + k2a_pk_lo(arg); b->max_q = (int)(argj & 0xffffu); }
		}
		b->rows = i0 + 2 * C;
		end_strip();
		return true;
	}

	K2A_FN void end_strip() { D = -1; kfin = kfinA = K2A_KNONE; rowsA_m1 = rowsB_m1 = -1; hasn = 0; }
};

template<int C>
K2A_FN int k2a_trace_solo(const uint8_t *tb, int i, int j, uint32_t *out, int qlen, int tlen, int w)
{
	enum { WB = 2 * C, AHEAD = 8 };
	int n = 0, state = 0;
	uint32_t last_op = 0xffffffffu, run = 0;
	const size_t nsteps = k2a_solo_steps<C>(qlen, tlen, w);
	while (i >= 0 && j >= 0) {
		const int D = i / (2 * C), r = i - D * 2 * C, half = r >= C ? 1 : 0, c = r - half * C;
		const uint8_t *p = tb + k2a_tb_word((size_t)(j + 2 * D + half), D % 64, nsteps, 64, WB) + 2 * c + half;
		const int nq = k2a_min(k2a_min(AHEAD, c + 1), k2a_min(i, j) + 1);
		uint32_t bq[AHEAD];
#pragma unroll
		for (int k = 0; k < AHEAD; ++k) bq[k] = p[-(ptrdiff_t)k2a_min(k, nq - 1) * (WB + 2)];
		bool diagonal = true;
#pragma unroll
		for (int k = 0; k < AHEAD; ++k) {
			if (k >= nq || !diagonal) break;
			const uint32_t d = k2a_flags_decode(bq[k]);
			if (state == 0) state = d & 7;
			else if (!((d >> (state + 2)) & 1)) state = 0;
			if (state == 0) state = d & 7;
			uint32_t op;
			if (state == 0) { op = 0; --i; --j; }
			else if (state == 1 || state == 3) { op = 2; --i; diagonal = false; }
			else { op = 1; --j; diagonal = false; }
			if (op == last_op) ++run;
			else { if (run) out[n++] = run << 4 | last_op; last_op = op; run = 1; }
		}
	}
	if (i >= 0) {
		if (last_op == 2) run += i + 1;
		else { if (run) out[n++] = run << 4 | last_op; last_op = 2; run = i + 1; }
// ... 11 lines not shown
```

### ksw2_amd/csrc/ksw2_shim_hip.hip

```cpp
#include <hip/hip_runtime.h>
#include <stdio.h>
#include <string.h>
#include "ksw2_shim.h"
#include "ksw2_lane.h"
#include "ksw2_lane_pk.h"
#include "ksw2_lane_pkmp.h"
#include "ksw2_lane_solo.h"
#include "ksw2_lane_dm.h"
#include "ksw2_lane_extf.h"
#include "ksw2_lane_ssec.h"
#include "ksw2_lane_ssecb.h"
#include "ksw2_lane_extfb.h"
#include "ksw2_lane_ll.h"
#include "ksw2_lane_llchk.h"
#include "ksw2_lane_llsub.h"

#define K2A_WPB 4
#define K2A_TRACE_PPW_MAX 8
static int k2a_trace_ppw(int nwalks)
{
	const int target_waves = 4096;
	int ppw = (nwalks + target_waves - 1) / target_waves;
	return ppw < 1 ? 1 : ppw > K2A_TRACE_PPW_MAX ? K2A_TRACE_PPW_MAX : ppw;
}
// ... 368 lines not shown
				}
			} else {
				const bool gfin = ((finmask >> (grp * G)) & (G == 64 ? ~0ull : (1ull << (G & 63)) - 1)) != 0;
				if (nfin) L.stage_rows(rowbuf);
				__builtin_amdgcn_wave_barrier();
				if (gfin) L.fin_local_rows(sc, rowbuf);
				if (nfin) L.end_strip();
				__builtin_amdgcn_wave_barrier();
			}
			if (TN && L.wn) K2A_SYNC_WN(L);
		}
		if (!NOSTOP && zseq && __builtin_amdgcn_ballot_w64(!(gdone || k >= klast)) == 0) { stop = true; break; }
	}
	L.qwA = qpa; L.qwB = qpb;
	}
	if (STAGED) ST.finish(kdone);
	__builtin_amdgcn_wave_barrier();
	if (!zseq) {
		uint32_t *loc = &stage_w[0];
		loc[lane * 5 + 0] = L.lmax; loc[lane * 5 + 1] = L.lmax_t; loc[lane * 5 + 2] = L.lmax_q;
		loc[lane * 5 + 3] = L.lmqe; loc[lane * 5 + 4] = L.lmqe_t;
		__builtin_amdgcn_wave_barrier();
		if (valid && gl == 0) {
			k2a_merge_local(loc + grp * G * 5, G, 0, bkA);
			k2a_merge_local(loc + grp * G * 5, G, 1, bkB);
			bkA->rows = bkB->rows = prA.tlen;
		}
		__builtin_amdgcn_wave_barrier();
		if (valid && prA.tlen == prA.tlen_full && gl == ((prA.tlen_full - 1) % C) % G) {
			const bool reach = prA.tlen_full - 1 + prA.w >= prA.qlen - 1;
			bkA->mte = k2a_pk_lo(L.last_m); bkA->mte_q = k2a_pk_lo(L.last_j);
			bkB->mte = k2a_pk_hi(L.last_m); bkB->mte_q = k2a_pk_hi(L.last_j);
			if (reach) { bkA->score = k2a_pk_lo(L.last_h); bkB->score = k2a_pk_hi(L.last_h); }
		}
		__builtin_amdgcn_wave_barrier();
	}
	const uint64_t sawmask = __builtin_amdgcn_ballot_w64(valid && (scan_on ? (scan & 2u) != 0 : L.saw_wildcard()));
	const bool gsaw = ((sawmask >> (grp * G)) & (G == 64 ? ~0ull : (1ull << (G & 63)) - 1)) != 0;
	if (valid && gl == 0) {
		const K2aBook a = *bkA, b = *bkB;
		k2a_finish(prA, a, &res[piA]);
		if (piB != piA) k2a_finish(prB, b, &res[piB]);
		if (gsaw) { res[piA].pad[0] = 1; res[piB].pad[0] = 1; }
	}
}

template<int G, int C, bool DUAL, int MODE, bool RB, bool NOMAX, int LDSROW = 0, bool DEFER = false, bool QUEUE = false>
__global__ void __launch_bounds__(64 * K2A_WPB, LDSROW == 2 ? (G == 16 ? 4 : 3) : LDSROW ? 2 : 1)
k2a_fill_pk_kernel(const K2aScoring sc, const K2aPair *__restrict__ pairs, const uint32_t *__restrict__ order2, int ntasks,
                   const uint8_t *__restrict__ seq, uint8_t *__restrict__ tb, K2aResult *__restrict__ res, K2aQueueDesc *qd)
{
	constexpr int NG = 64 / G;
	typedef K2aLanePk<G, C, DUAL, MODE, RB, NOMAX, LDSROW, DEFER, false> Lane;
	__shared__ K2aBook book[K2A_WPB][NG][2];
	__shared__ uint32_t stage[K2A_WPB][(NG * K2A_PK_STAGE(C) > 64 * 5) ? NG * K2A_PK_STAGE(C) : 64 * 5];

	const int lane = threadIdx.x & 63, wave = k2a_wave_id<(C <= 8 || LDSROW || (NOMAX && DUAL && MODE != K2A_MODE_SCORE))>();
	const int grp = lane / G, gl = lane % G;
	const int wt = blockIdx.x * K2A_WPB + wave;
	if (DEFER && blockIdx.x == 0 && threadIdx.x == 0) {
		uint32_t *zlist = (uint32_t*)(tb + pairs[order2[0]].tb_off) - K2A_ZLIST_WORDS(ntasks);
		__hip_atomic_store(&zlist[0], 0u, __ATOMIC_RELAXED, __HIP_MEMORY_SCOPE_AGENT);
	}
	if (QUEUE && !k2a_queue_wait(qd, wt)) return;
	constexpr int LROW_WORDS = LDSROW == 1 ? K2A_PK_LDSROW_WORDS(C) : LDSROW == 2 ? K2A_PK_LDSCODE_WORDS(C) : 0;
	__shared__ uint32_t lrows[LDSROW ? K2A_WPB * LROW_WORDS : 1];
	__shared__ uint32_t cptab[K2A_WPB][8];
	constexpr int WB = Lane::TBWORDS * 4;
	constexpr bool STAGED = MODE != K2A_MODE_SCORE && (WB == 16 || WB == 32);
	typedef K2aTbStage<STAGED ? WB : 16, K2A_PK_TB_NS(WB, LDSROW)> Stage;
	__shared__ uint4 tbstage[STAGED ? K2A_WPB * Stage::WORDS : 1];
	__shared__ unsigned long long tbruns[STAGED ? K2A_WPB * 64 : 1];
	const int task = wt * NG + grp;
	uint32_t scan = 0;
	const bool scan_on = sc.pk_tn1 != 0;
	if (scan_on && task < ntasks) {
		const K2aPair pa = pairs[order2[2 * task]], pb = pairs[order2[2 * task + 1]];
		scan = k2a_scan_codes<G>(seq + pa.toff, pa.tlen_full, gl) | k2a_scan_codes<G>(seq + pb.toff, pb.tlen_full, gl);
	}
	{
		const uint64_t m1 = __builtin_amdgcn_ballot_w64((scan & 1u) != 0), m2 = __builtin_amdgcn_ballot_w64((scan & 2u) != 0);
		const uint64_t gm = (G == 64 ? ~0ull : (1ull << (G & 63)) - 1) << (grp * G);
		scan = ((m1 & gm) ? 1u : 0u) | ((m2 & gm) ? 2u : 0u);
		if (m1 != 0)
			k2a_fill_pk_body<G, C, DUAL, MODE, RB, NOMAX, LDSROW, DEFER, true>(sc, pairs, order2, ntasks, seq, tb, res, wt, wave, lane, grp, gl, scan_on, scan, book, stage[wave], lrows, cptab, tbstage, tbruns);
		else
			k2a_fill_pk_body<G, C, DUAL, MODE, RB, NOMAX, LDSROW, DEFER, false>(sc, pairs, order2, ntasks, seq, tb, res, wt, wave, lane, grp, gl, scan_on, scan, book, stage[wave], lrows, cptab, tbstage, tbruns);
	}
}

template<int G, int C, bool RB>
__global__ void __launch_bounds__(64 * K2A_WPB)
k2a_argmax_kernel(const K2aScoring sc, const K2aPair *__restrict__ pairs, const uint32_t *__restrict__ order2, int ntasks,
                  const uint8_t *__restrict__ seq, uint8_t *__restrict__ ck, K2aResult *__restrict__ res, const K2aQueueDesc *qd)
{
	constexpr int NG = 64 / G;
	if (qd && (__hip_atomic_load(&qd->abort, __ATOMIC_RELAXED, __HIP_MEMORY_SCOPE_AGENT) != 0 ||
	           __hip_atomic_load(&qd->next, __ATOMIC_RELAXED, __HIP_MEMORY_SCOPE_AGENT) != qd->nwt)) return;
	typedef K2aLanePk<G, C, false, K2A_MODE_SCORE, RB, false, 0, false, true> Lane;
	const int job = blockIdx.x * (64 * K2A_WPB) + threadIdx.x;
	const int task = job / 3, which = job - 3 * task;
	bool go = task < ntasks;
	const bool live = go;
	const uint32_t piA = order2[go ? 2 * task : 0], piB = order2[go ? 2 * task + 1 : 0];
	const K2aPair prA = pairs[piA], prB = pairs[piB];
	const bool inexA = res[piA].pad[1] != 0, inexB = res[piB].pad[1] != 0;
	int row = -1;
	if (go) {
		if (which == 0) row = res[piA].max_t;
		else if (which == 1) row = piB == piA ? -1 : res[piB].max_t;
		else row = (prA.tlen == prA.tlen_full && !(inexA && inexB)) ? prA.tlen_full - 1 : -1;
	}
	go = go && row >= 0;
	const int S = go ? row / C : 0, grp = task % NG;
	__shared__ uint32_t cptab[K2A_WPB][8];
	k2a_cptab_fill(sc, cptab[threadIdx.x >> 6], (int)(threadIdx.x & 63));
	Lane L;
	L.lrow = 0;
	L.setup(prA, prB, seq, S % G, go, cptab[threadIdx.x >> 6]);
	L.Snext = S;
	L.schedule_next();
	const int kbeg = L.knext;
	const uint8_t *blk = ck + prA.tb_off;
	if (go) L.do_init(sc, 0, 0, (const K2aCkHead*)(blk + (size_t)prA.bnd_off * K2A_CK_STEP_BYTES) + (size_t)grp * prA.cig_off + S);
	K2A_SYNC_WN(L);
	const int n = go ? L.kfin - kbeg + 1 : 0;
	const uint2 *st = (const uint2*)blk + (grp * G + S % G);
	for (int t = 0; __builtin_amdgcn_ballot_w64(t < n) != 0; ++t) {
		if (t < n) {
			const int k = kbeg + t;
			const uint2 in = st[(size_t)k * 64];
			const int jc = min(max(k - L.koff, 0), L.qlen - 1);
			L.set_qb(k2a_pair16(L.qa[jc], L.qbp[jc]));
			uint32_t tw[Lane::TBWORDS];
			L.step(sc, k, in.x, in.y, 0u, tw);
		}
	}
	if (go) {
		const int c = row - S * C;
		k2a_pk v = 0;
#pragma unroll
		for (int cc = 0; cc < C; ++cc) if (cc == c) v = L.rmj(cc);
		if (which == 0) res[piA].max_q = (int)(v & 0xffffu);
		else if (which == 1) res[piB].max_q = (int)(v >> 16);
		else {
			if (!inexA) res[piA].mte_q = (int)(v & 0xffffu);
			if (piB != piA && !inexB) res[piB].mte_q = (int)(v >> 16);
		}
	}
	if (live && ((which == 0 && inexA) || (which == 1 && inexB && piB != piA))) {
		uint32_t *zlist = (uint32_t*)(ck + pairs[order2[0]].tb_off) - K2A_ZLIST_WORDS(ntasks);
		const uint32_t at = __hip_atomic_fetch_add(&zlist[0], 1u, __ATOMIC_RELAXED, __HIP_MEMORY_SCOPE_AGENT);
		zlist[1 + at] = (uint32_t)task * 2u + (uint32_t)which;
	}
}

template<int G, int C, bool RB>
__global__ void __launch_bounds__(64 * K2A_WPB)
k2a_zscan_kernel(const K2aScoring sc, const K2aPair *__restrict__ pairs, const uint32_t *__restrict__ order2, int ntasks,
                 const uint8_t *__restrict__ seq, const uint8_t *__restrict__ ck, K2aResult *__restrict__ res, const K2aQueueDesc *qd)
{
	constexpr int NG = 64 / G, ZG = 16, ZNG = 64 / ZG;
	if (qd && (__hip_atomic_load(&qd->abort, __ATOMIC_RELAXED, __HIP_MEMORY_SCOPE_AGENT) != 0 ||
	           __hip_atomic_load(&qd->next, __ATOMIC_RELAXED, __HIP_MEMORY_SCOPE_AGENT) != qd->nwt)) return;
	typedef K2aLanePk<G, C, false, K2A_MODE_SCORE, RB, false, 0, false, true> Lane;
	__shared__ uint32_t stage[K2A_WPB][64][K2A_PK_STAGE(C)];
	__shared__ K2aBook book[K2A_WPB][ZNG];
// ... 122 lines not shown
	for (int k = kg; k <= kge; ++k) {
		const k2a_pk rh = (k2a_pk)k2a_rot1<64>((int)L.hout);
		k2a_pk hin = __builtin_amdgcn_alignbit(L.hout, rh, 16);
		k2a_pk ein = __builtin_amdgcn_alignbit(L.eout, (k2a_pk)k2a_rot1<64>((int)L.eout), 16);
		k2a_pk e2in = DUAL ? __builtin_amdgcn_alignbit(L.e2out, (k2a_pk)k2a_rot1<64>((int)L.e2out), 16) : 0u;

		const bool ninit = L.need_init(k);
		if (__builtin_amdgcn_ballot_w64(ninit) != 0) {
			const int bs = k2a_rot1<64>(L.baseB);
			if (ninit) L.do_init(sc, bs);
			if (TN) K2A_SYNC_WN(L);
		}
		const bool nhigh = L.need_init_high(k);
		if (__builtin_amdgcn_ballot_w64(nhigh) != 0) {
			if (nhigh) L.start_high(sc);
		}
		L.hu_prev = rh;
		hin = k2a_pk_add(hin, L.delta); ein = k2a_pk_add(ein, L.delta); if (DUAL) e2in = k2a_pk_add(e2in, L.delta);
		L.advance_query(k & 3);
		if (k <= ktop) L.top_inputs(sc, k, hin, ein, e2in);

		uint32_t tw[Lane::TBWORDS];
		const bool live = L.step(sc, k, hin, ein, e2in, tw);
		if (STAGED) { ST.put(k, tw, live); ST.step_done(k); kdone = k; }
		else if (MODE != K2A_MODE_SCORE) {
			if (live) {
				uint32_t *dst = (uint32_t*)(tbp + k2a_tb_word((size_t)k, lane, tbsteps, 64, Lane::TBWORDS * 4));
#pragma unroll
				for (int x = 0; x + 3 < Lane::TBWORDS; x += 4) *(uint4*)(dst + x) = make_uint4(tw[x], tw[x + 1], tw[x + 2], tw[x + 3]);
				if (Lane::TBWORDS & 2) *(uint2*)(dst + (Lane::TBWORDS & ~3)) = make_uint2(tw[Lane::TBWORDS & ~3], tw[(Lane::TBWORDS & ~3) + 1]);
			}
		}
		const bool nsave = L.need_save(k);
		if (__builtin_amdgcn_ballot_w64(nsave) != 0) {
			if (nsave) L.save_low();
		}
		const bool nfin = L.need_fin(k);
		if (__builtin_amdgcn_ballot_w64(nfin) != 0) {
			const bool slow = nfin && !L.fin_fast(sc, bk, pr.zdrop);
			if (__builtin_amdgcn_ballot_w64(slow) != 0) {
				if (slow) { L.stage_rows(stage[wave]); L.do_fin_seq(sc, bk, pr.zdrop, stage[wave]); }
				__builtin_amdgcn_wave_barrier();
				if (bk->dropped) { stop = true; break; }
			}
			if (TN && L.wn) K2A_SYNC_WN(L);
		}
	}
	L.qw = qp;
	}
	if (STAGED) ST.finish(kdone);
	__builtin_amdgcn_wave_barrier();
	const bool saw = scan_on ? (scan & 2u) != 0 : __builtin_amdgcn_ballot_w64(valid && L.saw_wildcard()) != 0;
	if (valid && lane == 0) {
		const K2aBook b = *bk;
		k2a_finish(pr, b, &res[pi]);
		if (saw) res[pi].pad[0] = 1;
	}
}

template<int C, bool DUAL, int MODE>
__global__ void __launch_bounds__(64 * K2A_WPB)
k2a_fill_solo_kernel(const K2aScoring sc, const K2aPair *__restrict__ pairs, const uint32_t *__restrict__ order, int ntasks,
                     const uint8_t *__restrict__ seq, uint8_t *__restrict__ tb, K2aResult *__restrict__ res)
{
	typedef K2aLaneSolo<C, DUAL, MODE, false> Lane;
	constexpr int WB = Lane::TBWORDS * 4;
	constexpr bool STAGED = MODE != K2A_MODE_SCORE && (WB == 16 || WB == 32);
	typedef K2aTbStage<STAGED ? WB : 16, 8> Stage;
	__shared__ K2aBook book[K2A_WPB];
	__shared__ uint32_t stage[K2A_WPB][K2A_SOLO_STAGE(C)];
	__shared__ uint32_t cptab[K2A_WPB][8];
	__shared__ uint4 tbstage[STAGED ? K2A_WPB * Stage::WORDS : 1];
	__shared__ unsigned long long tbruns[STAGED ? K2A_WPB * 64 : 1];
	const int lane = threadIdx.x & 63, wave = k2a_wave_id<true>();
	const int task = blockIdx.x * K2A_WPB + wave;
	const bool scan_on = sc.pk_tn1 != 0;
	uint32_t scan = 0;
	if (scan_on && task < ntasks) {
		const K2aPair pr = pairs[order[task]];
		scan = k2a_scan_codes<64>(seq + pr.toff, pr.tlen_full, lane);
	}
	const bool any4 = __builtin_amdgcn_ballot_w64((scan & 1u) != 0) != 0;
	scan = (any4 ? 1u : 0u) | (__builtin_amdgcn_ballot_w64((scan & 2u) != 0) != 0 ? 2u : 0u);
	if (any4) k2a_fill_solo_body<C, DUAL, MODE, true>(sc, pairs, order, ntasks, seq, tb, res, task, wave, lane, scan_on, scan, book, stage, cptab, tbstage, tbruns);
	else k2a_fill_solo_body<C, DUAL, MODE, false>(sc, pairs, order, ntasks, seq, tb, res, task, wave, lane, scan_on, scan, book, stage, cptab, tbstage, tbruns);
}

template<int C>
__global__ void __launch_bounds__(64)
k2a_trace_solo_kernel(const K2aPair *__restrict__ pairs, const uint32_t *__restrict__ order, int ntasks,
                      const uint8_t *__restrict__ tb, K2aResult *__restrict__ res, uint32_t *__restrict__ cig, int ppw)
{
	if ((int)threadIdx.x >= ppw) return;
	const int t = blockIdx.x * ppw + threadIdx.x;
	if (t >= ntasks) return;
	const uint32_t pi = order[t];
	const K2aPair pr = pairs[pi];
	const int ti = res[pi].ti, tj = res[pi].tj;
	int n = 0;
	if (ti >= 0 && tj >= 0) n = k2a_trace_solo<C>(tb + pr.tb_off, ti, tj, cig + pr.cig_off, pr.qlen, pr.tlen, pr.w);
	res[pi].n_cigar = n;
}

template<int G, int C, bool DUAL, int MODE, bool LROW = false>
__global__ void __launch_bounds__(64 * K2A_WPB, LROW ? 2 : 1)
k2a_fill_mp_kernel(const K2aScoring sc, const K2aPair *__restrict__ pairs, const uint32_t *__restrict__ order, int ntasks,
                   const uint8_t *__restrict__ seq, uint8_t *__restrict__ tb, int32_t *bnd, K2aResult *__restrict__ res)
{
	static_assert(G == 64, "one alignment per wavefront");
	typedef K2aLane<G, C, DUAL, MODE, LROW> Lane;
	__shared__ K2aBook book[K2A_WPB];
	__shared__ int rowbuf[K2A_WPB][3 * C];
	__shared__ int lrows[LROW ? K2A_WPB * K2A_LROW_WORDS(C) : 1];
	__shared__ uint32_t tabs[16];
	__shared__ int8_t mtab[K2A_MAXM * K2A_MAXM];
	if (threadIdx.x < 5) { tabs[threadIdx.x] = sc.prof[threadIdx.x]; tabs[8 + threadIdx.x] = (uint32_t)sc.colw[threadIdx.x]; }
	if (sc.m > 5) for (int x = threadIdx.x; x < sc.m * sc.m; x += blockDim.x) mtab[x] = sc.mat[x];
	__syncthreads();

	const int gl = threadIdx.x & 63, wave = k2a_wave_id<true>();
	const int task = blockIdx.x * K2A_WPB + wave;
	const bool valid = task < ntasks;
	const uint32_t pi = order[valid ? task : 0];
	const K2aPair pr = pairs[pi];

	Lane L;
	L.lrow = &lrows[LROW ? wave * K2A_LROW_WORDS(C) + gl : 0];
	L.setup(pr, seq, gl, valid);
	K2aBook *bk = &book[wave];
	if (gl == 0) k2a_book_reset(bk);
	__builtin_amdgcn_wave_barrier();

	int32_t *Bh = bnd + pr.bnd_off, *Be = Bh + pr.qlen, *Be2 = Be + pr.qlen;
	uint8_t *tbp = tb + pr.tb_off;
	const size_t tbsteps = (MODE != K2A_MODE_SCORE && valid) ? k2a_tb_steps<G, C, true>(pr.qlen, pr.tlen, pr.w) : 0;
	const int R = G * C;
	const int ngen = valid ? (pr.tlen + R - 1) / R : 0;
	size_t kbase = 0;
	bool dropped = false;
	const int ktop = __builtin_amdgcn_readfirstlane(valid ? min(pr.qlen - 1, min(C - 1, pr.tlen - 1) + pr.w) : -1);

	for (int g = 0; g < ngen && !dropped; ++g) {
		int jlo, nsteps;
		k2a_gen_cols<G, C>(g, pr.qlen, pr.tlen, pr.w, &jlo, &nsteps);
		L.begin_generation(g, jlo);
		const bool feeder = (gl == 0 && g > 0);
		const bool drain = (gl == G - 1);
		int ph0 = K2A_NEG, pe0 = K2A_NEG, pe20 = K2A_NEG, ph1 = K2A_NEG, pe1 = K2A_NEG, pe21 = K2A_NEG;
		if (feeder) {
			if (jlo > 0) L.hu_prev = __hip_atomic_load(&Bh[jlo - 1], __ATOMIC_RELAXED, __HIP_MEMORY_SCOPE_AGENT);
			ph0 = __hip_atomic_load(&Bh[jlo], __ATOMIC_RELAXED, __HIP_MEMORY_SCOPE_AGENT);
			pe0 = __hip_atomic_load(&Be[jlo], __ATOMIC_RELAXED, __HIP_MEMORY_SCOPE_AGENT);
			if (DUAL) pe20 = __hip_atomic_load(&Be2[jlo], __ATOMIC_RELAXED, __HIP_MEMORY_SCOPE_AGENT);
			if (jlo + 1 < pr.qlen) {
				ph1 = __hip_atomic_load(&Bh[jlo + 1], __ATOMIC_RELAXED, __HIP_MEMORY_SCOPE_AGENT);
				pe1 = __hip_atomic_load(&Be[jlo + 1], __ATOMIC_RELAXED, __HIP_MEMORY_SCOPE_AGENT);
				if (DUAL) pe21 = __hip_atomic_load(&Be2[jlo + 1], __ATOMIC_RELAXED, __HIP_MEMORY_SCOPE_AGENT);
			}
		}
		L.qb = L.next_query_code(-1);
		for (int k = 0; k < nsteps; ++k) {
			int hin = k2a_rot1<G>(L.hout);
			int ein = k2a_rot1<G>(L.eout);
			int e2in = DUAL ? k2a_rot1<G>(L.e2out) : 0;
			if (feeder) {
				hin = ph0; ein = pe0; e2in = pe20;
				ph0 = ph1; pe0 = pe1; pe20 = pe21;
// ... 236 lines not shown
					if (ninit) L.do_init(sc, bsA, bsB);
					bsA = k2a_rot1<G>(L.P.baseA); bsB = k2a_rot1<G>(L.P.baseB);
					L.refresh_delta(bsA, bsB);
					if (TN) K2A_SYNC_WN(L.P);
				}
				if (feeder) {
					take(jlo + k, cur, cur2);
					hin = cur.x; ein = cur.y; e2in = cur2;
					L.refresh_delta((int)cur.z, (int)cur.w);
				}
				cur = nxt; cur2 = nxt2;
				fetch_raw(jlo + k + 2, nxt, nxt2);
				L.P.hu_prev = hin;
				hin = L.adopt(hin); ein = L.adopt(ein);
				if (DUAL) e2in = L.adopt(e2in);
				const uint32_t qnext = L.P.next_query_codes(k);
				if (g == 0 && k <= ktop) L.P.top_inputs(sc, k, hin, ein, e2in);
				uint32_t tw[Lane::TBWORDS];
				const int jj = L.column(k);
				const bool mine = L.P.S >= 0 && jj >= 0 && jj <= L.P.je;
				const bool live = L.P.step(sc, k, hin, ein, e2in, tw);
				if (STAGED) { ST.put(kbase + k, tw, live); ST.step_done(kbase + k); kdone = k; }
				if (drain && mine) {
					B1[jj] = make_uint4(L.P.hout, L.P.eout, (uint32_t)L.P.baseA, (uint32_t)L.P.baseB);
					if (DUAL) B2[jj] = L.P.e2out;
				}
				const bool nfin = L.need_fin(k);
				if (__builtin_amdgcn_ballot_w64(nfin) != 0) {
					if (nfin) L.flush_rowmax();
					__builtin_amdgcn_fence(__ATOMIC_RELEASE, "workgroup");
					if (nfin) L.do_fin(sc, bkA, bkB, zdropA, zdropB, rowbuf[wave]);
					__builtin_amdgcn_wave_barrier();
					if (TN && L.P.wn) K2A_SYNC_WN(L.P);
				}
				L.P.set_qb(qnext);
				if ((k & (T - 1)) == T - 1) {
					const k2a_pk d = L.rebase();
					const k2a_pk da = (k2a_pk)k2a_rot1<G>((int)d);
					const int bsA = k2a_rot1<G>(L.P.baseA), bsB = k2a_rot1<G>(L.P.baseB);
					L.after_rebase(da, bsA, bsB);
				}
			}
			if (k1 == nsteps) {
				if (STAGED && kdone >= 0) ST.finish(kbase + kdone);
				g += W;
			}
		}
		__builtin_amdgcn_fence(__ATOMIC_RELEASE, "workgroup");
		__syncthreads();
		__builtin_amdgcn_fence(__ATOMIC_ACQUIRE, "workgroup");
	}
	__syncthreads();
	if (threadIdx.x == 0) {
		const K2aBook a = *bkA, b = *bkB;
		k2a_finish(prA, a, &res[piA]);
		if (piB != piA) k2a_finish(prB, b, &res[piB]);
	}
}

template<bool DUAL, int MODE>
__global__ void __launch_bounds__(64 * K2A_PKMP_WAVES, K2A_PKMP_WAVES > 4 ? 3 : 2)
k2a_fill_pkmp_kernel(const K2aScoring sc, const K2aPair *__restrict__ pairs, const uint32_t *__restrict__ order2, int ntasks,
                     const uint8_t *__restrict__ seq, uint8_t *__restrict__ tb, uint32_t *bnd, K2aResult *__restrict__ res)
{
	constexpr int C = 16, W = K2A_PKMP_WAVES;
	typedef K2aLanePkMp<C, DUAL, MODE, false> Lane;
	constexpr int WB = Lane::TBWORDS * 4;
	constexpr bool STAGED = MODE != K2A_MODE_SCORE;
	typedef K2aTbStage<WB, 8> Stage;
	__shared__ K2aBook book[2];
	__shared__ uint32_t rowbuf[W][C];
	__shared__ int pstart[64 + 1], pcount[64];
	__shared__ uint4 tbstage[STAGED ? W * Stage::WORDS : 1];
	__shared__ unsigned long long tbruns[STAGED ? W * 64 : 1];
	__shared__ uint32_t cptab[W][8];
	const int lane = threadIdx.x & 63, wave = __builtin_amdgcn_readfirstlane((int)(threadIdx.x >> 6));
	const int task = blockIdx.x;
	if (task >= ntasks) return;
	uint32_t scan = 0;
	if (sc.pk_tn1) {
		const K2aPair pa = pairs[order2[2 * task]], pb = pairs[order2[2 * task + 1]];
		scan = k2a_scan_codes<64>(seq + pa.toff, pa.tlen_full, lane) | k2a_scan_codes<64>(seq + pb.toff, pb.tlen_full, lane);
	}
	if (__builtin_amdgcn_ballot_w64((scan & 1u) != 0) != 0)
		k2a_fill_pkmp_body<DUAL, MODE, true>(sc, pairs, order2, ntasks, seq, tb, bnd, res, task, wave, lane, book, rowbuf, pstart, pcount, tbstage, tbruns, cptab);
	else
		k2a_fill_pkmp_body<DUAL, MODE, false>(sc, pairs, order2, ntasks, seq, tb, bnd, res, task, wave, lane, book, rowbuf, pstart, pcount, tbstage, tbruns, cptab);
}


__device__ __forceinline__ int k2a_shr1_carry(int v, int carry)
{
	return __builtin_amdgcn_update_dpp(carry, v, 0x138 , 0xf, 0xf, false);
}

template<int CTRL>
__device__ __forceinline__ uint64_t k2a_dpp_max_u64(uint64_t k)
{
	const uint32_t lo = (uint32_t)__builtin_amdgcn_update_dpp(0, (int)(uint32_t)k, CTRL, 0xf, 0xf, false);
	const uint32_t hi = (uint32_t)__builtin_amdgcn_update_dpp(0, (int)(uint32_t)(k >> 32), CTRL, 0xf, 0xf, false);
	const uint64_t o = ((uint64_t)hi << 32) | lo;
	return o > k ? o : k;
}
template<int CTRL>
__device__ __forceinline__ uint32_t k2a_dpp_max_u32(uint32_t v)
{
	const uint32_t o = (uint32_t)__builtin_amdgcn_update_dpp(0, (int)v, CTRL, 0xf, 0xf, false);
	return o > v ? o : v;
}
__device__ __forceinline__ uint32_t k2a_wave_max_u32(uint32_t v)
{
	v = k2a_dpp_max_u32<0x121>(v);
	v = k2a_dpp_max_u32<0x122>(v);
	v = k2a_dpp_max_u32<0x124>(v);
	v = k2a_dpp_max_u32<0x128>(v);
	const uint32_t a = (uint32_t)__builtin_amdgcn_readlane((int)v, 0), b = (uint32_t)__builtin_amdgcn_readlane((int)v, 16);
	const uint32_t c = (uint32_t)__builtin_amdgcn_readlane((int)v, 32), d = (uint32_t)__builtin_amdgcn_readlane((int)v, 48);
	const uint32_t ab = a > b ? a : b, cd = c > d ? c : d;
	return ab > cd ? ab : cd;
}
__device__ __forceinline__ uint64_t k2a_wave_max_u64(uint64_t k)
{
	const uint32_t hi = (uint32_t)(k >> 32), lo = (uint32_t)k;
	const uint32_t M = k2a_wave_max_u32(hi);
	const uint32_t L = k2a_wave_max_u32(hi == M ? lo : 0u);
	return ((uint64_t)M << 32) | L;
}

template<int MODE, int K>
__global__ void __launch_bounds__(64 * K2A_WPB)
k2a_exts_kernel(const K2aSplice sp, const K2aPair *__restrict__ pairs, const uint32_t *__restrict__ order, int ntasks,
                const uint8_t *__restrict__ seq, uint8_t *__restrict__ tb, K2aResult *__restrict__ res)
{
	__shared__ int8_t mtab[K2A_MAXM * K2A_MAXM];
	__shared__ int hrow[K2A_WPB][K * 64];
	for (int x = threadIdx.x; x < sp.m * sp.m; x += blockDim.x) mtab[x] = sp.mat[x];
	__syncthreads();

	const int lane = threadIdx.x & 63, wave = k2a_wave_id<true>();
	const int task = blockIdx.x * K2A_WPB + wave;
	if (task >= ntasks) return;
	int *const hw = hrow[wave];
	const uint32_t pi = order[task];
	const K2aPair pr = pairs[pi];
	const int qlen = pr.qlen, tlen = pr.tlen_full, ncol = min(qlen, tlen);
	const uint8_t *qry = seq + pr.qoff;
	const uint32_t *cst = (const uint32_t*)seq + pr.bnd_off;
	uint8_t *tbp = tb + pr.tb_off;

	int H1[K], H2[K], En[K], E2n[K], Fn[K];
	uint32_t Q[K], Cst[K];
#pragma unroll
	for (int s = 0; s < K; ++s) {
		H1[s] = H2[s] = En[s] = E2n[s] = Fn[s] = K2A_NEG; Q[s] = 0;
		Cst[s] = cst[min(s * 64 + lane, tlen - 1)];
	}
	int base = 0;
	K2aBook book;
	k2a_book_reset(&book);
	uint32_t qnext = qry[0];

	for (int r = 0; r < qlen + tlen - 1; ++r) {
		const int st0 = max(0, r - qlen + 1), en0 = min(tlen - 1, r), en1 = st0 + (en0 - st0) / 4 * 4;
		if (st0 >= 1 && (st0 - 1) / 64 > base) {
#pragma unroll
			for (int s = 0; s + 1 < K; ++s) {
				H1[s] = H1[s + 1]; H2[s] = H2[s + 1]; En[s] = En[s + 1]; E2n[s] = E2n[s + 1]; Fn[s] = Fn[s + 1]; Q[s] = Q[s + 1]; Cst[s] = Cst[s + 1];
// ... 1470 lines not shown
```

### ksw2_amd/csrc/ksw2_types.h

```cpp
#ifndef KSW2_TYPES_H_
#define KSW2_TYPES_H_

#include <stdint.h>

#define K2A_NEG      (-0x40000000)
#define K2A_KNONE    0x7fffffff
#define K2A_MAXM     127

#define K2A_F_SCORE_ONLY 0x01
#define K2A_F_EXTZ_ONLY 0x40
#define K2A_F_REV_CIGAR 0x80
#define K2A_F_SPLICE_FOR   0x100
#define K2A_F_SPLICE_REV   0x200
#define K2A_F_SPLICE_FLANK 0x400
#define K2A_F_HAS_JUNC     0x10000000

#define K2A_MODE_SCORE 0
#define K2A_MODE_LEFT  1
#define K2A_MODE_RIGHT 2

#define K2A_TB_PAD 32
#define K2A_TB_PADDED(steps) (((steps) + (K2A_TB_PAD - 1)) / K2A_TB_PAD * K2A_TB_PAD)

#define K2A_NEG16    (-16384)
#define K2A_OFS16    0x4C00
#define K2A_PK_VMAX  (0x7BFF - K2A_OFS16)
#define K2A_PK_SLACK (K2A_OFS16 + K2A_NEG16)
#ifndef K2A_PKMP_T
#define K2A_PKMP_T    64
#endif
#define K2A_PKMP_DEAD (-8192)
#define K2A_PKMP_RMAX_LIMIT 10000
#define K2A_PK_NIBBLES(C, dual) (!(dual) && (C) == 16)
#define K2A_PK_TB_BYTES(C, dual) (K2A_PK_NIBBLES(C, dual) ? (C) : 2 * (C))

typedef struct K2aScoring {
	int32_t q, e, q2, e2;
	uint32_t prof[5];
	int32_t colw[5];
	uint32_t cp[8];
	int32_t pk_smax;
	int32_t pk_tn1;
	int32_t m;
	const int8_t *mat;
} K2aScoring;

#define K2A_DM_SLOTS_S 8
#define K2A_DM_SLOTS   16
#define K2A_DM_DIAG(K) ((K) * 64 - 64)

typedef struct K2aSplice {
	int32_t q, e, q2, long_thres;
	int32_t m;
	const int8_t *mat;
} K2aSplice;

typedef struct K2aExtf {
	int32_t mch, mis, e;
	int32_t ring;
} K2aExtf;
#define K2A_EXTF_RING_ROWS(span) (((span) + 30) / 4 + 3)

typedef struct K2aSsec {
	int32_t q, e, q2, e2;
	int32_t qe_first;
	int32_t long_thres, long_diff;
	int32_t m, sc_mch, sc_mis, sc_N;
	const int8_t *mat;
} K2aSsec;
#define K2A_SSEC_APPROX      1
#define K2A_SSEC_APPROX_DROP 2
#define K2A_SSEC_GENERIC     4

#define K2A_EXTF_WIN_SPAN(K) (64 * (K) - 109)

typedef struct K2aPair {
	uint32_t qoff, toff;
	int32_t qlen, tlen;
	int32_t tlen_full;
	int32_t w;
	int32_t zdrop, end_bonus, flag;
	uint32_t cig_off;
	uint64_t tb_off;
	uint32_t bnd_off;
	uint32_t pad;
} K2aPair;

typedef struct K2aResult {
	int32_t max, zdropped, max_q, max_t, mqe, mqe_t, mte, mte_q, score, reach_end, n_cigar, rows_done;
	int32_t ti, tj;
	int32_t pad[2];
} K2aResult;

#define K2A_WM_BYTES 65536
#define K2A_WIRE2_ESC 7
#define K2A_WIRE2_SLOT (4 * K2A_WIRE2_ESC)
#define K2A_WIRE2_PAD (4 * K2A_WIRE2_SLOT)

typedef struct K2aQueueDesc {
	uint32_t next;
	uint32_t abort;
	uint32_t nwt;
	uint32_t unp_fmt;
	const uint32_t *need;
	const uint32_t *wm;
	uint64_t timeout_ticks;
	const uint8_t *unp_src;
	uint8_t *unp_dst;
	uint32_t unp_bytes, unp_total;
} K2aQueueDesc;

#define K2A_ZLIST_WORDS(ntasks) ((2 * (size_t)(ntasks) + 16 + 63) & ~(size_t)63)

#define K2A_UNI_MAXPIECES 48
typedef struct K2aUniform {
	K2aPair tmpl;
	uint32_t n, ntasks, ng;
	uint32_t stride, qpad;
	uint32_t defer;
	uint64_t blk_base, blk_bytes;
	uint32_t npieces, margin;
	uint64_t seq_bytes;
	uint64_t pb[K2A_UNI_MAXPIECES + 1];
} K2aUniform;

typedef struct K2aBook {
	int32_t max, max_t, max_q, mqe, mqe_t, mte, mte_q, score, dropped, rows;
// ... 40 lines not shown
```

Measured before the change: 5062 GCUPS.

## Store hl pre-offset by gap-open so candidate needs one add instead of add+sub

Adds a K2A_HL_OPEN mode, on by default, in which the per-row hl state is kept shifted by q. The packed score profile is precomputed as q+e+score minus a base. The inner diagonal candidate then becomes a single add of a permuted profile byte instead of add-bias-then-subtract, and hl stores the pre-max value t. Borders, rebasing, and end/score readouts are compensated by hq. When the base is nonzero the TN-fix path is forced on, which can add a per-cell correction and disable the cheaper non-TN template variant.

```diff
diff --git a/ksw2_amd/csrc/ksw2_host_plan.c b/ksw2_amd/csrc/ksw2_host_plan.c
--- a/ksw2_amd/csrc/ksw2_host_plan.c
+++ b/ksw2_amd/csrc/ksw2_host_plan.c
@@ -340,7 +340,7 @@
 	}
 }
 
-typedef struct { int ok, smax, smin, qemax, qemin, q, e, tn1; uint32_t cp[8]; } pkinfo_t;
+typedef struct { int ok, smax, smin, qemax, qemin, q, e, tn1, base, tnc; uint32_t cp[8]; } pkinfo_t;
 
 static void pk_scoring(int dual, int m, const int8_t *mat, int q, int e, int q2, int e2, int generic, pkinfo_t *o)
 {
@@ -351,11 +351,22 @@
 		build_eff(dual, m, mat, e, e2, generic, eff);
 		o->smax = o->smin = eff[0];
 		for (x = 0; x < m * m; ++x) { o->smax = imax(o->smax, eff[x]); o->smin = imin(o->smin, eff[x]); }
+#if K2A_HL_OPEN
+		{
+			int lo = 0x7fffffff, hi = -0x7fffffff;
+			for (y = 0; y < m; ++y)
+				for (x = 0; x < 4 && x < m; ++x) { lo = imin(lo, q + e + eff[x * m + y]); hi = imax(hi, q + e + eff[x * m + y]); }
+			o->base = lo < 0 ? lo : hi > 255 ? hi - 255 : 0;
+			for (y = 0; y < m; ++y)
+				for (x = 0; x < 4 && x < m; ++x) o->cp[y] |= (uint32_t)(q + e + eff[x * m + y] - o->base) << (8 * x);
+		}
+#else
 		for (y = 0; y < m; ++y)
 			for (x = 0; x < 4 && x < m; ++x) o->cp[y] |= (uint32_t)(o->smax - eff[x * m + y]) << (8 * x);
+#endif
 		if (m == 5 && !(ENV(TN) && ENV(TN)[0] == '0')) {
 			for (y = 1; y < 5 && eff[4 * 5 + y] == eff[4 * 5]; ++y) {}
-			if (y == 5) o->tn1 = o->smax - eff[4 * 5] + 1;
+			if (y == 5) { o->tn1 = o->smax - eff[4 * 5] + 1; o->tnc = q + e + eff[4 * 5] - o->base; }
 		}
 	}
 	o->q = q; o->e = e;
@@ -865,7 +876,7 @@
 			c->cfg = c->solo ? 0 : pass ? (pass - 1) % K2A_NPKCFG : ci / 6; c->rb = pass && !c->solo ? ((pass - 1) / K2A_NPKCFG) & 1 : 0;
 			c->nomax = !c->solo && pass > 2 * K2A_NPKCFG; c->mode = (ci / 2) % 3; c->generic = ci & 1; c->pk = pass != 0 && !c->solo; c->first = k;
 			build_scoring(dual, m, sc->mat, q, e, q2, e2, c->generic, &c->sc);
-			if (pkinfo[c->generic].ok > 0) { memcpy(c->sc.cp, pkinfo[c->generic].cp, sizeof(c->sc.cp)); c->sc.pk_smax = pkinfo[c->generic].smax; c->sc.pk_tn1 = pkinfo[c->generic].tn1; }
+			if (pkinfo[c->generic].ok > 0) { memcpy(c->sc.cp, pkinfo[c->generic].cp, sizeof(c->sc.cp)); c->sc.pk_smax = pkinfo[c->generic].smax; c->sc.pk_tn1 = pkinfo[c->generic].tn1; c->sc.pk_base = pkinfo[c->generic].base; c->sc.pk_tnc = pkinfo[c->generic].tnc; }
 			if (uni) {
 				if (!pass || c->solo) { for (i = 0; i < cnt; ++i) p->h_order[k++] = (uint32_t)i; ntask = cnt; }
 				else for (i = 0; i < cnt; i += 2, ++ntask) { p->h_order[k++] = (uint32_t)i; p->h_order[k++] = (uint32_t)(i + 1 < cnt ? i + 1 : i); }
@@ -1471,9 +1482,10 @@
 		const int G = k->solo ? 64 : k->pk ? k2a_pkcfg_G[k->cfg] : k2a_cfg_G[k->cfg], C = k->solo ? 2 * K2A_SOLO_ROWS(k->mode == K2A_MODE_SCORE) : k->pk ? k2a_pkcfg_C[k->cfg] : k2a_cfg_C[k->cfg];
 		const int form = k->defer ? 3 : k->solo ? 0 : k->pk ? (k->cfg == K2A_PKCFG_MP ? 0 : k2a_shim_pk_form(k->cfg, p->dual, k->mode, k->nomax, k->count))
 		                                     : (k->cfg == K2A_CFG_MP ? k2a_shim_mp_form(p->dual, k->mode, k->count) : 0);
-		len += snprintf(buf + len, (size_t)(cap - len), "kernel=%s G=%d C=%d gaps=%d mode=%s rebased=%d nomax=%d generic=%d form=%s tasks=%d uniform=%d wire4=%d tn=%d\n",
+		len += snprintf(buf + len, (size_t)(cap - len), "kernel=%s G=%d C=%d gaps=%d mode=%s rebased=%d nomax=%d generic=%d form=%s tasks=%d uniform=%d wire4=%d tn=%d base=%d\n",
 		                kind, G, C, p->dual ? 2 : 1, mode_name[k->mode], k->rb, k->nomax, k->generic, form_name[form], k->count, p->uni ? 1 : 0,
-		                p->up_state ? p->up_state->wire4 : 0, (k->pk || k->solo) && k->sc.pk_tn1 ? 1 : 0);
+		                p->up_state ? p->up_state->wire4 : 0, (k->pk || k->solo) && k->sc.pk_tn1 ? 1 : 0,
+		                (k->pk || k->solo) ? k->sc.pk_base : 0);
 	}
 	return p->ncls;
 }
diff --git a/ksw2_amd/csrc/ksw2_lane_pk.h b/ksw2_amd/csrc/ksw2_lane_pk.h
--- a/ksw2_amd/csrc/ksw2_lane_pk.h
+++ b/ksw2_amd/csrc/ksw2_lane_pk.h
@@ -122,11 +122,21 @@
 	const uint32_t n = x & 0x00040004u;
 	return ((x ^ n) + K2A_TSEL_BASE) | n | (n << 1);
 }
-K2A_FN k2a_pk k2a_tn_fix(k2a_pk cand, uint32_t sel, int tn1)
+K2A_FN k2a_pk k2a_tn_fix(k2a_pk cand, uint32_t sel, const K2aScoring &sc)
 {
 	const uint32_t m = (sel >> 3) & 0x00010001u;
-	return cand - m * ((uint32_t)(tn1 - 1) & 0xffu);
-}
+#if K2A_HL_OPEN
+	return k2a_pk_add(k2a_pk_add(cand, k2a_pk2(sc.pk_base)), m * ((uint32_t)sc.pk_tnc & 0xffffu));
+#else
+	return cand - m * ((uint32_t)(sc.pk_tn1 - 1) & 0xffu);
+#endif
+}
+#if defined(__HIP_DEVICE_COMPILE__)
+#define K2A_TN_PATH(TN) (TN)
+#else
+#define K2A_TN_PATH(TN) true
+#endif
+K2A_FN int k2a_hl_q(const K2aScoring &sc) { return K2A_HL_OPEN ? sc.q : 0; }
 
 #define K2A_SGN_SEL 0x09080b0au
 template<bool DUAL, bool NIBBLE, bool INV>
@@ -274,7 +284,7 @@
 		const int js = k2a_max(0, i0 - w);
 		const k2a_pk neg = k2a_pku(K2A_NEG16);
 		const uint8_t *tpa = ta + (size_t)S * C, *tpb = tbq + (size_t)S * C;
-		hasn = 0;
+		hasn = (K2A_TN_PATH(TN) && K2A_HL_OPEN && sc.pk_base != 0) ? 1u : 0u;
 #pragma unroll
 		for (int c4 = 0; c4 < C; c4 += 4) {
 			uint32_t da, db;
@@ -296,9 +306,10 @@
 			if (!NOMAX) set_rmax(c, neg);
 		}
 		const int hcorner = k2a_border<DUAL>(sc, i0) + sc.e * (i0 - 1);
+		const int hq = k2a_hl_q(sc);
 		if (forced) { baseA = forced->baseA; baseB = forced->baseB; delta = 0; }
 		else if (RB) {
-			const int nbA = js == 0 ? hcorner : bsA + k2a_pk_lo(k2a_ofs_off(hu_prev)), nbB = js == 0 ? hcorner : bsB + k2a_pk_hi(k2a_ofs_off(hu_prev));
+			const int nbA = js == 0 ? hcorner : bsA + hq + k2a_pk_lo(k2a_ofs_off(hu_prev)), nbB = js == 0 ? hcorner : bsB + hq + k2a_pk_hi(k2a_ofs_off(hu_prev));
 			delta = S == 0 ? 0u : k2a_pair16((uint32_t)(bsA - nbA) & 0xffffu, (uint32_t)(bsB - nbB) & 0xffffu);
 			baseA = nbA; baseB = nbB;
 		}
@@ -309,16 +320,16 @@
 				for (int c = 0; c < C; ++c) {
 					const int hb = k2a_border<DUAL>(sc, i0 + c + 1) + sc.e * (i0 + c);
 					if (i0 + c <= w) {
-						hl[c] = k2a_ofs_on(k2a_pair16((uint32_t)(hb - baseA) & 0xffffu, (uint32_t)(hb - baseB) & 0xffffu));
-						f[c] = k2a_pk_sub(hl[c], k2a_pk2(sc.q + sc.e));
-						if (DUAL) f2[c] = k2a_pk_sub(hl[c], k2a_pk2(sc.q2 + sc.e2));
+						hl[c] = k2a_ofs_on(k2a_pair16((uint32_t)(hb - hq - baseA) & 0xffffu, (uint32_t)(hb - hq - baseB) & 0xffffu));
+						f[c] = k2a_pk_sub(hl[c], k2a_pk2(sc.q + sc.e - hq));
+						if (DUAL) f2[c] = k2a_pk_sub(hl[c], k2a_pk2(sc.q2 + sc.e2 - hq));
 					}
 				}
 			}
 		}
 		if (forced) hd0 = forced->hd0;
-		else if (RB) hd0 = K2A_OFS;
-		else if (js == 0) hd0 = k2a_pku(hcorner);
+		else if (RB) hd0 = k2a_pku(-hq);
+		else if (js == 0) hd0 = k2a_pku(hcorner - hq);
 		else hd0 = hu_prev;
 		Snext += G;
 		schedule_next();
@@ -329,7 +340,7 @@
 		if (S == 0) {
 			const int hb = k2a_border<DUAL>(sc, k - koff + 1);
 			const k2a_pk h0 = k2a_ofs_on(k2a_pair16((uint32_t)(hb - baseA) & 0xffffu, (uint32_t)(hb - baseB) & 0xffffu));
-			hin = k2a_pk_sub(h0, k2a_pk2(sc.e));
+			hin = k2a_pk_sub(h0, k2a_pk2(sc.e + k2a_hl_q(sc)));
 			ein = k2a_pk_sub(h0, k2a_pk2(sc.q + sc.e)); e2in = k2a_pk_sub(h0, k2a_pk2(sc.q2 + sc.e2));
 		}
 	}
@@ -346,7 +357,9 @@
 		const int dd = k - kd;
 		const k2a_pk neg = k2a_pku(K2A_NEG16);
 		const k2a_pk gq = k2a_pk2(sc.q), ge = k2a_pk2(sc.e), gq2 = k2a_pk2(sc.q2), ge2 = k2a_pk2(sc.e2), de2 = k2a_pk2(sc.e2 - sc.e);
+#if !K2A_HL_OPEN
 		const k2a_pk bias = k2a_pk2(sc.pk_smax + sc.e);
+#endif
 		k2a_pk e = ein, e2 = e2in;
 		if (dd >= wup) { e = neg; e2 = neg; }
 		rp.begin(dd, w, rows_m1);
@@ -361,11 +374,15 @@
 			for (int r = 0; r < CH; ++r) {
 				const int c = c0 + r;
 				const k2a_pk up = r == 0 ? above_old : hl[c - 1];
+#if K2A_HL_OPEN
+				cand[r] = k2a_add32(up, k2a_perm(cpB, cpA, tc(c)));
+#else
 				cand[r] = k2a_sub32(k2a_add32(up, bias), k2a_perm(cpB, cpA, tc(c)));
+#endif
 			}
-			if (TN && wn) {
-#pragma unroll
-				for (int r = 0; r < CH; ++r) cand[r] = k2a_tn_fix(cand[r], tc(c0 + r), sc.pk_tn1);
+			if (K2A_TN_PATH(TN) && wn) {
+#pragma unroll
+				for (int r = 0; r < CH; ++r) cand[r] = k2a_tn_fix(cand[r], tc(c0 + r), sc);
 			}
 			above_old = last_old;
 			if (CH < C) K2A_SCHED_FENCE();
@@ -415,7 +432,7 @@
 						else uprev = u;
 					} else tbw[c >> 1] = k2a_perm(fl, dprev, 0x05040100u);
 				}
-				hl[c] = h;
+				hl[c] = K2A_HL_OPEN ? t : h;
 			}
 			if (CH < C) K2A_SCHED_FENCE();
 		}
@@ -481,7 +498,7 @@
 				if (i < tlen && !bdrop) {
 					const bool reach = i + w >= qlen - 1;
 					const int unb = (half ? baseB : baseA) - sc.e * i;
-					const int hend = (int)(int16_t)(rowbuf[c] >> sh) + unb, H = (int)(int16_t)(rowbuf[C + c] >> sh) + unb;
+					const int hend = (int)(int16_t)(rowbuf[c] >> sh) + k2a_hl_q(sc) + unb, H = (int)(int16_t)(rowbuf[C + c] >> sh) + unb;
 					const int j = (int)(uint16_t)(rowbuf[2 * C + c] >> sh);
 					if (reach && hend > bmqe) { bmqe = hend; bmqe_t = i; }
 					if (i == tlen_full - 1) { bmte = H; bmte_q = j; }
@@ -551,7 +568,7 @@
 			const int i = fi0 + c;
 			const k2a_pk bias = k2a_pk2(sc.e * i);
 			const k2a_pk pj = rowbuf[2 * C + c], ipk = k2a_pk2(i);
-			const k2a_pk ph = (i < tlen) ? k2a_pk_sub(rowbuf[c], bias) : k2a_pk2(K2A_NEG16);
+			const k2a_pk ph = (i < tlen) ? k2a_pk_sub(rowbuf[c], k2a_pk2(sc.e * i - k2a_hl_q(sc))) : k2a_pk2(K2A_NEG16);
 			const k2a_pk pm = (i < tlen) ? k2a_pk_sub(rowbuf[C + c], bias) : k2a_pk2(K2A_NEG16);
 			const k2a_pk up = k2a_pk_sign(k2a_pk_sub(lmax, pm));
 			lmax_t = k2a_pk_sel(up, ipk, lmax_t);
@@ -573,8 +590,8 @@
 			k2a_pk v = 0;
 #pragma unroll
 			for (int c = 0; c < C; ++c) if (i0 + c == last) v = k2a_ofs_off(hl[c]);
-			bA->score = k2a_pk_lo(v) + (RB ? baseA : 0) - sc.e * last;
-			bB->score = k2a_pk_hi(v) + (RB ? baseB : 0) - sc.e * last;
+			bA->score = k2a_pk_lo(v) + k2a_hl_q(sc) + (RB ? baseA : 0) - sc.e * last;
+			bB->score = k2a_pk_hi(v) + k2a_hl_q(sc) + (RB ? baseB : 0) - sc.e * last;
 		}
 		end_strip();
 	}
@@ -592,7 +609,7 @@
 		if (i < tlen && !bdrop) {
 			const bool reach = i + w >= qlen - 1;
 			const int unb = base - sc.e * i;
-			const int hend = (int)(int16_t)(rowbuf[c] >> sh) + unb, H = (int)(int16_t)(rowbuf[C + c] >> sh) + unb;
+			const int hend = (int)(int16_t)(rowbuf[c] >> sh) + k2a_hl_q(sc) + unb, H = (int)(int16_t)(rowbuf[C + c] >> sh) + unb;
 			const int j = (int)(uint16_t)(rowbuf[2 * C + c] >> sh);
 			if (reach && hend > bmqe) { bmqe = hend; bmqe_t = i; }
 			if (i == tlen_full - 1) { bmte = H; bmte_q = j; }
diff --git a/ksw2_amd/csrc/ksw2_lane_pkmp.h b/ksw2_amd/csrc/ksw2_lane_pkmp.h
--- a/ksw2_amd/csrc/ksw2_lane_pkmp.h
+++ b/ksw2_amd/csrc/ksw2_lane_pkmp.h
@@ -132,7 +132,7 @@
 				if (i < P.tlen && !bdrop) {
 					const bool reach = i + P.w >= P.qlen - 1;
 					const unsigned long long key = k2a_key_load(&spill[2 * c + half]);
-					const int hend = (int)(int16_t)(rowbuf[c] >> sh) + base - sc.e * i;
+					const int hend = (int)(int16_t)(rowbuf[c] >> sh) + k2a_hl_q(sc) + base - sc.e * i;
 					const int H = (int)((uint32_t)(key >> 32) ^ 0x80000000u) - sc.e * i;
 					const int j = FIRSTJ ? 0xffff - (int)(key & 0xffffu) : (int)(key & 0xffffu);
 					if (reach && hend > bmqe) { bmqe = hend; bmqe_t = i; }
diff --git a/ksw2_amd/csrc/ksw2_lane_solo.h b/ksw2_amd/csrc/ksw2_lane_solo.h
--- a/ksw2_amd/csrc/ksw2_lane_solo.h
+++ b/ksw2_amd/csrc/ksw2_lane_solo.h
@@ -100,7 +100,7 @@
 		wupA = w + (D == 0 ? 1 : 0);
 		const int js = k2a_max(0, i0 - w);
 		const k2a_pk neg = k2a_pku(K2A_NEG16);
-		hasn = 0;
+		hasn = (K2A_TN_PATH(TN) && K2A_HL_OPEN && sc.pk_base != 0) ? 1u : 0u;
 #pragma unroll
 		for (int c4 = 0; c4 < C; c4 += 4) {
 			const uint32_t da = tnA[c4 / 4], db = tnB[c4 / 4];
@@ -117,24 +117,25 @@
 #pragma unroll
 		for (int c = 0; c < C; ++c) { hl[c] = neg; f[c] = neg; if (DUAL) f2[c] = neg; rmax[c] = neg; rmj[c] = 0; }
 		const int hcorner = k2a_border<DUAL>(sc, i0) + sc.e * (i0 - 1);
-		const int nb = js == 0 ? hcorner : bs + k2a_pk_hi(k2a_ofs_off(hu_prev));
+		const int hq = k2a_hl_q(sc);
+		const int nb = js == 0 ? hcorner : bs + hq + k2a_pk_hi(k2a_ofs_off(hu_prev));
 		delta = D == 0 ? 0u : ((uint32_t)(bs - nb) & 0xffffu);
 		baseA = nb;
 		if (i0 <= w) {
 #pragma unroll
 			for (int c = 0; c < C; ++c) {
 				const int ha = k2a_border<DUAL>(sc, i0 + c + 1) + sc.e * (i0 + c);
-				const uint32_t va = i0 + c <= w ? k2a_h16(ha - baseA) : k2a_h16(K2A_NEG16);
+				const uint32_t va = i0 + c <= w ? k2a_h16(ha - hq - baseA) : k2a_h16(K2A_NEG16);
 				hl[c] = k2a_pair16(va, neg >> 16);
-				const k2a_pk fl = k2a_pk_sub(hl[c], k2a_pk2(sc.q + sc.e));
+				const k2a_pk fl = k2a_pk_sub(hl[c], k2a_pk2(sc.q + sc.e - hq));
 				f[c] = k2a_pair16(i0 + c <= w ? fl & 0xffffu : neg & 0xffffu, neg >> 16);
 				if (DUAL) {
-					const k2a_pk fl2 = k2a_pk_sub(hl[c], k2a_pk2(sc.q2 + sc.e2));
+					const k2a_pk fl2 = k2a_pk_sub(hl[c], k2a_pk2(sc.q2 + sc.e2 - hq));
 					f2[c] = k2a_pair16(i0 + c <= w ? fl2 & 0xffffu : neg & 0xffffu, neg >> 16);
 				}
 			}
 		}
-		hd0 = k2a_pair16(k2a_h16(0), neg >> 16);
+		hd0 = k2a_pair16(k2a_h16(-hq), neg >> 16);
 		qw = qn0 << qn_sh;
 		Dnext += G;
 		schedule_next();
@@ -145,7 +146,7 @@
 
 	K2A_FN void start_high(const K2aScoring &sc)
 	{
-		const int i0b = i0 + C;
+		const int i0b = i0 + C, hq = k2a_hl_q(sc);
 		if (i0b <= w) {
 			const uint32_t negh = (uint32_t)k2a_h16(K2A_NEG16);
 			baseB = k2a_border<DUAL>(sc, i0b) + sc.e * (i0b - 1);
@@ -153,7 +154,7 @@
 			for (int c = 0; c < C; ++c) {
 				const bool in = i0b + c <= w;
 				const int hb = k2a_border<DUAL>(sc, i0b + c + 1) + sc.e * (i0b + c) - baseB;
-				const uint32_t vb = in ? k2a_h16(hb) : negh;
+				const uint32_t vb = in ? k2a_h16(hb - hq) : negh;
 				const uint32_t fb = in ? k2a_h16(hb - (sc.q + sc.e)) : negh;
 				hl[c] = (hl[c] & 0xffffu) | (vb << 16);
 				f[c] = (f[c] & 0xffffu) | (fb << 16);
@@ -162,8 +163,8 @@
 					f2[c] = (f2[c] & 0xffffu) | (fb2 << 16);
 				}
 			}
-		} else baseB = baseA + k2a_pk_hi(k2a_ofs_off(hd0));
-		hd0 = (hd0 & 0xffffu) | ((uint32_t)k2a_h16(0) << 16);
+		} else baseB = baseA + hq + k2a_pk_hi(k2a_ofs_off(hd0));
+		hd0 = (hd0 & 0xffffu) | ((uint32_t)k2a_h16(-hq) << 16);
 		delta = (delta & 0xffffu) | (((uint32_t)(baseA - baseB) & 0xffffu) << 16);
 	}
 
@@ -171,7 +172,7 @@
 	{
 		if (D == 0) {
 			const int hb = k2a_border<DUAL>(sc, k - koff + 1) - baseA;
-			const uint32_t h0 = k2a_h16(hb - sc.e), e0 = k2a_h16(hb - (sc.q + sc.e));
+			const uint32_t h0 = k2a_h16(hb - sc.e - k2a_hl_q(sc)), e0 = k2a_h16(hb - (sc.q + sc.e));
 			const uint32_t e20 = k2a_h16(hb - (sc.q2 + sc.e2));
 			hin = (hin & 0xffff0000u) | h0; ein = (ein & 0xffff0000u) | e0; e2in = (e2in & 0xffff0000u) | e20;
 		}
@@ -182,7 +183,9 @@
 		const int ddA = k - kd, ddB = ddA - C - 1;
 		const k2a_pk neg = k2a_pku(K2A_NEG16);
 		const k2a_pk gq = k2a_pk2(sc.q), ge = k2a_pk2(sc.e), gq2 = k2a_pk2(sc.q2), ge2 = k2a_pk2(sc.e2), de2 = k2a_pk2(sc.e2 - sc.e);
+#if !K2A_HL_OPEN
 		const k2a_pk bias = k2a_pk2(sc.pk_smax + sc.e);
+#endif
 		const k2a_pk cut = k2a_pair16(ddA >= wupA ? 0xffffu : 0u, ddB >= w ? 0xffffu : 0u);
 		k2a_pk e = k2a_pk_sel(cut, neg, ein), e2 = DUAL ? k2a_pk_sel(cut, neg, e2in) : 0u;
 		const int loA = k2a_max(0, ddA - w), hiA = k2a_min(rowsA_m1, ddA + w), cntA = k <= kfinA ? k2a_max(hiA - loA + 1, 0) : 0;
@@ -199,11 +202,15 @@
 #pragma unroll
 			for (int r = 0; r < CH; ++r) {
 				const int c = c0 + r;
+#if K2A_HL_OPEN
+				cand[r] = k2a_add32(r == 0 ? above_old : hl[c - 1], k2a_perm(cpB, cpA, tc[c]));
+#else
 				cand[r] = k2a_sub32(k2a_add32(r == 0 ? above_old : hl[c - 1], bias), k2a_perm(cpB, cpA, tc[c]));
-			}
-			if (TN && wn) {
-#pragma unroll
-				for (int r = 0; r < CH; ++r) cand[r] = k2a_tn_fix(cand[r], tc[c0 + r], sc.pk_tn1);
+#endif
+			}
+			if (K2A_TN_PATH(TN) && wn) {
+#pragma unroll
+				for (int r = 0; r < CH; ++r) cand[r] = k2a_tn_fix(cand[r], tc[c0 + r], sc);
 			}
 			above_old = last_old;
 			if (CH < C) K2A_SCHED_FENCE();
@@ -245,7 +252,7 @@
 					if (c & 1) tbw[c >> 1] = k2a_perm(fl, dprev, 0x05040100u);
 					else dprev = fl;
 				}
-				hl[c] = h;
+				hl[c] = K2A_HL_OPEN ? t : h;
 			}
 			if (CH < C) K2A_SCHED_FENCE();
 		}
@@ -296,7 +303,7 @@
 			if (i < tlen && !bdrop) {
 				const bool reach = i + w >= qlen - 1;
 				const int unb = (c < C ? baseA : baseB) - sc.e * i;
-				const int hend = (int)(int16_t)rowbuf[c] + unb, H = (int)(int16_t)rowbuf[2 * C + c] + unb;
+				const int hend = (int)(int16_t)rowbuf[c] + k2a_hl_q(sc) + unb, H = (int)(int16_t)rowbuf[2 * C + c] + unb;
 				const int j = (int)(uint16_t)rowbuf[4 * C + c];
 				if (reach && hend > bmqe) { bmqe = hend; bmqe_t = i; }
 				if (i == tlen_full - 1) { bmte = H; bmte_q = j; }
diff --git a/ksw2_amd/csrc/ksw2_shim_hip.hip b/ksw2_amd/csrc/ksw2_shim_hip.hip
--- a/ksw2_amd/csrc/ksw2_shim_hip.hip
+++ b/ksw2_amd/csrc/ksw2_shim_hip.hip
@@ -474,7 +474,7 @@
 		const uint64_t m1 = __builtin_amdgcn_ballot_w64((scan & 1u) != 0), m2 = __builtin_amdgcn_ballot_w64((scan & 2u) != 0);
 		const uint64_t gm = (G == 64 ? ~0ull : (1ull << (G & 63)) - 1) << (grp * G);
 		scan = ((m1 & gm) ? 1u : 0u) | ((m2 & gm) ? 2u : 0u);
-		if (m1 != 0)
+		if (m1 != 0 || sc.pk_base != 0)
 			k2a_fill_pk_body<G, C, DUAL, MODE, RB, NOMAX, LDSROW, DEFER, true>(sc, pairs, order2, ntasks, seq, tb, res, wt, wave, lane, grp, gl, scan_on, scan, book, stage[wave], lrows, cptab, tbstage, tbruns);
 		else
 			k2a_fill_pk_body<G, C, DUAL, MODE, RB, NOMAX, LDSROW, DEFER, false>(sc, pairs, order2, ntasks, seq, tb, res, wt, wave, lane, grp, gl, scan_on, scan, book, stage[wave], lrows, cptab, tbstage, tbruns);
@@ -763,7 +763,7 @@
 	}
 	const bool any4 = __builtin_amdgcn_ballot_w64((scan & 1u) != 0) != 0;
 	scan = (any4 ? 1u : 0u) | (__builtin_amdgcn_ballot_w64((scan & 2u) != 0) != 0 ? 2u : 0u);
-	if (any4) k2a_fill_solo_body<C, DUAL, MODE, true>(sc, pairs, order, ntasks, seq, tb, res, task, wave, lane, scan_on, scan, book, stage, cptab, tbstage, tbruns);
+	if (any4 || sc.pk_base != 0) k2a_fill_solo_body<C, DUAL, MODE, true>(sc, pairs, order, ntasks, seq, tb, res, task, wave, lane, scan_on, scan, book, stage, cptab, tbstage, tbruns);
 	else k2a_fill_solo_body<C, DUAL, MODE, false>(sc, pairs, order, ntasks, seq, tb, res, task, wave, lane, scan_on, scan, book, stage, cptab, tbstage, tbruns);
 }
 
@@ -1166,7 +1166,7 @@
 		const K2aPair pa = pairs[order2[2 * task]], pb = pairs[order2[2 * task + 1]];
 		scan = k2a_scan_codes<64>(seq + pa.toff, pa.tlen_full, lane) | k2a_scan_codes<64>(seq + pb.toff, pb.tlen_full, lane);
 	}
-	if (__builtin_amdgcn_ballot_w64((scan & 1u) != 0) != 0)
+	if (__builtin_amdgcn_ballot_w64((scan & 1u) != 0) != 0 || sc.pk_base != 0)
 		k2a_fill_pkmp_body<DUAL, MODE, true>(sc, pairs, order2, ntasks, seq, tb, bnd, res, task, wave, lane, book, rowbuf, pstart, pcount, tbstage, tbruns, cptab);
 	else
 		k2a_fill_pkmp_body<DUAL, MODE, false>(sc, pairs, order2, ntasks, seq, tb, bnd, res, task, wave, lane, book, rowbuf, pstart, pcount, tbstage, tbruns, cptab);
diff --git a/ksw2_amd/csrc/ksw2_types.h b/ksw2_amd/csrc/ksw2_types.h
--- a/ksw2_amd/csrc/ksw2_types.h
+++ b/ksw2_amd/csrc/ksw2_types.h
@@ -31,6 +31,9 @@
 #endif
 #define K2A_PKMP_DEAD (-8192)
 #define K2A_PKMP_RMAX_LIMIT 10000
+#ifndef K2A_HL_OPEN
+#define K2A_HL_OPEN 1
+#endif
 #define K2A_PK_NIBBLES(C, dual) (!(dual) && (C) == 16)
 #define K2A_PK_TB_BYTES(C, dual) (K2A_PK_NIBBLES(C, dual) ? (C) : 2 * (C))
 
@@ -43,6 +46,7 @@
 	int32_t pk_tn1;
 	int32_t m;
 	const int8_t *mat;
+	int32_t pk_base, pk_tnc;
 } K2aScoring;
 
 #define K2A_DM_SLOTS_S 8
```

Result: faster. 5338 GCUPS (median of 6 runs) (+5.5%).
